# byteowlz/kokorox

Hardware: NVIDIA B200
Metric: audio-seconds per second (higher is better)
Workload: dtype bf16

## Files before the change

kokorox_b200/csrc/capi.cu:

```cuda
#include "../../include/kkx.h"
#include "../../include/kkx_test.h"
#include "model.h"
#include <chrono>
#include <condition_variable>
#include <cstring>
#include <deque>
#include <mutex>
#include <map>
#include <numeric>
#include <set>
#include <sstream>
#include <atomic>
#include <thread>

using namespace kkx;

struct kkx_ctx {
  std::unique_ptr<Model> model;
  std::mutex mu;
  std::mutex pool_mu;
  std::map<float*, size_t> pinned;
  std::vector<std::pair<float*, size_t>> pinned_free;
  size_t pinned_free_floats = 0;
  size_t pinned_hi = 0;
// ... 445 lines not shown
    if (law != 0 && law != 1) throw ArgError("law must be 0 (mu-law) or 1 (A-law), got " + std::to_string(law));
    Model& m = *ctx->model;
    m.stage(batch, tokens, tok_offsets, styles, speeds);
    m.set_g711(law);
    try { m.run(); } catch (...) { m.set_g711(-1); throw; }
    m.set_g711(-1);
    const long long n = m.total_samples();
    size_t cap = 0;
    float* host = take_pinned(ctx, (size_t)(n + 3) / 4, &cap);
    try {
      m.fetch_g711(reinterpret_cast<unsigned char*>(host), n, out_sample_offsets, out_pred_dur);
    } catch (...) { cudaFreeHost(host); throw; }
    hand_out(ctx, host, cap);
    *out_codes = reinterpret_cast<uint8_t*>(host);
  });
}

KKX_API void kkx_release_g711(kkx_ctx* ctx, uint8_t* codes) { kkx_release(ctx, reinterpret_cast<float*>(codes)); }

KKX_API int kkx_infer_batch_flac(kkx_ctx* ctx, int32_t batch, const int64_t* tokens, const int32_t* tok_offsets,
                                 const float* styles, const float* speeds, uint8_t** out_bytes,
                                 int64_t* out_byte_offsets, int64_t* out_sample_offsets, int32_t* out_pred_dur) {
  int rc = check_ctx(ctx);
  if (rc) return rc;
  if (out_bytes) *out_bytes = nullptr;
  std::lock_guard<std::mutex> lk(ctx->mu);
  return guarded(ctx, [&] {
    if (!out_bytes) throw ArgError("out_bytes is null");
    if (!out_byte_offsets) throw ArgError("out_byte_offsets is null");
    Model& m = *ctx->model;
    m.stage(batch, tokens, tok_offsets, styles, speeds);
    m.set_pcm16(true);
    try { m.run(); } catch (...) { m.set_pcm16(false); throw; }
    m.set_pcm16(false);
    m.encode_flac();
    const long long n = m.flac_bytes();
    size_t cap = 0;
    float* host = take_pinned(ctx, (size_t)(n + 3) / 4, &cap);
    try {
      m.fetch_flac(reinterpret_cast<unsigned char*>(host), n, out_byte_offsets, out_sample_offsets, out_pred_dur);
    } catch (...) { cudaFreeHost(host); throw; }
    hand_out(ctx, host, cap);
    *out_bytes = reinterpret_cast<uint8_t*>(host);
  });
}

KKX_API void kkx_release_flac(kkx_ctx* ctx, uint8_t* bytes) { kkx_release(ctx, reinterpret_cast<float*>(bytes)); }

static void put_u16(uint8_t* p, uint32_t v) { p[0] = (uint8_t)v; p[1] = (uint8_t)(v >> 8); }
static void put_u32(uint8_t* p, uint32_t v) { put_u16(p, v & 0xFFFF); put_u16(p + 2, v >> 16); }
static void wav_header(uint8_t* h, uint32_t riff_size, uint32_t data_size, uint32_t format, uint32_t channels,
                       uint32_t rate, uint32_t bits) {
  memcpy(h, "RIFF", 4); put_u32(h + 4, riff_size); memcpy(h + 8, "WAVEfmt ", 8);
  put_u32(h + 16, 16); put_u16(h + 20, format); put_u16(h + 22, channels); put_u32(h + 24, rate);
  put_u32(h + 28, rate * channels * bits / 8); put_u16(h + 32, channels * bits / 8); put_u16(h + 34, bits);
  memcpy(h + 36, "data", 4); put_u32(h + 40, data_size);
}

KKX_API int32_t kkx_wav_header_pcm16(uint8_t* dst44, int64_t n_samples, int32_t sample_rate) {
  if (!dst44 || n_samples < 0 || sample_rate <= 0) return KKX_ERR_ARG;
  const uint32_t bytes = (uint32_t)(n_samples * 2);
  wav_header(dst44, 36u + bytes, bytes, 1, 1, (uint32_t)sample_rate, 16);
  return 44;
}

KKX_API int32_t kkx_wav_header_f32_stream(uint8_t* dst44, int32_t channels, int32_t sample_rate) {
  if (!dst44 || channels <= 0 || sample_rate <= 0) return KKX_ERR_ARG;
  wav_header(dst44, 0xFFFFFFFFu, 0xFFFFFFFFu, 3, (uint32_t)channels, (uint32_t)sample_rate, 32);
  return 44;
}

KKX_API int64_t kkx_encode_wav16_base64(const int16_t* pcm, int64_t n_samples, int32_t sample_rate, char* dst,
                                int64_t capacity) {
  if (n_samples < 0 || sample_rate <= 0 || (!pcm && n_samples > 0)) return KKX_ERR_ARG;
  const int64_t nbytes = 44 + n_samples * 2;
  const int64_t nchars = (nbytes + 2) / 3 * 4;
  if (!dst || capacity < nchars) return nchars;
  static const char T[] = "ABCDEFGHIJKLMNOPQRSTUVWXYZabcdefghijklmnopqrstuvwxyz0123456789+/";
  uint8_t head[48];
  kkx_wav_header_pcm16(head, n_samples, sample_rate);
  const uint8_t* body = reinterpret_cast<const uint8_t*>(pcm);
  const int64_t nbody = n_samples * 2;
  const int borrow = (int)std::min<int64_t>(4, nbody);
  for (int i = 0; i < borrow; i++) head[44 + i] = body[i];
  const int hbytes = 44 + borrow;
  char* o = dst;
  auto group = [&](const uint8_t* p, int n) {
    const uint32_t v = ((uint32_t)p[0] << 16) | ((n > 1 ? (uint32_t)p[1] : 0u) << 8) | (n > 2 ? (uint32_t)p[2] : 0u);
    o[0] = T[v >> 18]; o[1] = T[(v >> 12) & 63];
    o[2] = n > 1 ? T[(v >> 6) & 63] : '=';
    o[3] = n > 2 ? T[v & 63] : '=';
    o += 4;
  };
  int hp = 0;
  for (; hp + 3 <= hbytes; hp += 3) group(head + hp, 3);
  if (hp < hbytes) {
    group(head + hp, hbytes - hp);
  } else {
    int64_t bp = borrow;
    for (; bp + 3 <= nbody; bp += 3) group(body + bp, 3);
    if (bp < nbody) group(body + bp, (int)(nbody - bp));
  }
  if (capacity > nchars) *o = 0;
  return nchars;
}

KKX_API int kkx_infer(kkx_ctx* ctx, const int64_t* tokens, int32_t n_tokens, const float* style256,
              float speed, float** out_audio, int64_t* out_samples, int32_t* out_pred_dur) {
  if (out_samples) *out_samples = 0;
  if (ctx && ctx->model && ctx->coalesce_max.load() > 1) {
    if (out_audio) *out_audio = nullptr; else { g_err = "out_audio is null"; return KKX_ERR_ARG; }
    const int vrc = validate_request(tokens, n_tokens, style256, speed);
    if (vrc != KKX_OK) return vrc;
    kkx_ctx::Waiter w{tokens, n_tokens, style256, speed, out_pred_dur};
    const int rc = infer_coalesced(ctx, w);
    if (rc == KKX_OK) { *out_audio = w.audio; if (out_samples) *out_samples = w.samples; }
    return rc;
  }
  const int32_t offs[2] = {0, n_tokens};
  int64_t soff[2] = {0, 0};
  const int rc = kkx_infer_batch(ctx, 1, tokens, offs, style256, &speed, out_audio, soff, out_pred_dur);
  if (rc == KKX_OK && out_samples) *out_samples = soff[1];
  return rc;
}

static void async_worker(kkx_ctx* ctx) {
  std::unique_lock<std::mutex> al(ctx->amu);
  for (;;) {
    ctx->acv_work.wait(al, [&] { return ctx->astop || !ctx->aqueue.empty(); });
    if (ctx->astop) {
      for (auto* r : ctx->aqueue) { r->w.rc = KKX_ERR_STATE; r->w.err = "session destroyed before the request ran"; r->done = true; }
      ctx->aqueue.clear();
      ctx->acv_done.notify_all();
      return;
    }
    std::vector<kkx_ctx::AsyncReq*> reqs;
    std::vector<kkx_ctx::Waiter*> batch;
    long long tok = 0;
    const size_t want = (size_t)std::max(ctx->async_batch.load(), 1);
    while (!ctx->aqueue.empty() && reqs.size() < want) {
      kkx_ctx::AsyncReq* r = ctx->aqueue.front();
      if (!reqs.empty() && tok + r->w.n > 64 * 512) break;
      tok += r->w.n;
      reqs.push_back(r);
      batch.push_back(&r->w);
      ctx->aqueue.pop_front();
    }
    al.unlock();
    try {
      serve_coalesced(ctx, batch, false);
    } catch (...) {
      for (auto* w : batch) { w->rc = KKX_ERR_CUDA; w->err = "internal error while serving an asynchronous batch"; w->audio = nullptr; }
    }
    al.lock();
    ctx->async_batches++;
    ctx->async_requests += (int64_t)reqs.size();
    for (auto* r : reqs) r->done = true;
    ctx->acv_done.notify_all();
  }
}

KKX_API int kkx_submit(kkx_ctx* ctx, const int64_t* tokens, int32_t n_tokens, const float* style256, float speed,
                       kkx_ticket* out_ticket) {
  int rc = check_ctx(ctx);
  if (rc) return rc;
  if (!out_ticket) { g_err = "out_ticket is null"; return KKX_ERR_ARG; }
  *out_ticket = 0;
  rc = validate_request(tokens, n_tokens, style256, speed);
  if (rc) return rc;
  try {
    std::unique_ptr<kkx_ctx::AsyncReq> r(new kkx_ctx::AsyncReq());
    r->tokens.assign(tokens, tokens + n_tokens);
    memcpy(r->style, style256, sizeof r->style);
    r->dur.assign((size_t)n_tokens, 0);
    r->w.tokens = r->tokens.data(); r->w.n = n_tokens; r->w.style = r->style; r->w.speed = speed;
    r->w.pred_dur = r->dur.data();
    std::lock_guard<std::mutex> al(ctx->amu);
    if (ctx->astop) { g_err = "Session is not initialized."; return KKX_ERR_STATE; }
    if (!ctx->worker_started) {
      ctx->worker = std::thread(async_worker, ctx);
      ctx->worker_started = true;
    }
    const int64_t t = ctx->next_ticket++;
    ctx->aqueue.push_back(r.get());
    ctx->tickets[t] = std::move(r);
    *out_ticket = t;
  } catch (const std::exception& e) { g_err = e.what(); return KKX_ERR_CUDA; }
  ctx->acv_work.notify_one();
  return KKX_OK;
}

KKX_API int kkx_poll(kkx_ctx* ctx, kkx_ticket ticket) {
  int rc = check_ctx(ctx);
  if (rc) return rc;
  std::lock_guard<std::mutex> al(ctx->amu);
  auto it = ctx->tickets.find(ticket);
  if (it == ctx->tickets.end() || it->second->taken) { g_err = "unknown ticket"; return KKX_ERR_ARG; }
  return it->second->done ? 1 : 0;
}

KKX_API int kkx_wait(kkx_ctx* ctx, kkx_ticket ticket, float** out_audio, int64_t* out_samples, int32_t* out_pred_dur) {
  int rc = check_ctx(ctx);
  if (rc) return rc;
  if (out_audio) *out_audio = nullptr;
  if (out_samples) *out_samples = 0;
  std::unique_ptr<kkx_ctx::AsyncReq> r;
  {
    std::unique_lock<std::mutex> al(ctx->amu);
    auto it = ctx->tickets.find(ticket);
    if (it == ctx->tickets.end() || it->second->taken) { g_err = "unknown ticket"; return KKX_ERR_ARG; }
    it->second->taken = true;
    kkx_ctx::AsyncReq* p = it->second.get();
    ctx->acv_done.wait(al, [&] { return p->done; });
    r = std::move(it->second);
    ctx->tickets.erase(it);
  }
  if (r->w.rc != KKX_OK) { g_err = r->w.err; return r->w.rc; }
  if (out_pred_dur) memcpy(out_pred_dur, r->dur.data(), r->dur.size() * sizeof(int32_t));
  if (out_samples) *out_samples = r->w.samples;
  if (out_audio) *out_audio = r->w.audio; else kkx_release(ctx, r->w.audio);
  return KKX_OK;
}

KKX_API void kkx_release(kkx_ctx* ctx, float* audio) {
  if (!ctx || !audio) return;
  float* to_free = nullptr;
  {
    std::lock_guard<std::mutex> pl(ctx->pool_mu);
    auto vit = ctx->views.find(audio);
    if (vit != ctx->views.end()) {
      kkx_ctx::SharedBuf* sb = vit->second;
      ctx->views.erase(vit);
      if (--sb->refs > 0) return;
      ctx->pinned[sb->base] = sb->cap;
      audio = sb->base;
      delete sb;
    }
    auto it = ctx->pinned.find(audio);
    if (it == ctx->pinned.end()) return;
    if (ctx->pinned_free.size() < 64 && ctx->pinned_free_floats + it->second <= (size_t(1) << 28)) {
      ctx->pinned_free.push_back({it->first, it->second});
      ctx->pinned_free_floats += it->second;
    } else {
      to_free = audio;
    }
    ctx->pinned.erase(it);
  }
  if (to_free) {
    if (ctx->model) cudaSetDevice(ctx->model->device());
    cudaFreeHost(to_free);
  }
}

KKX_API int kkx_stage_batch(kkx_ctx* ctx, int32_t batch, const int64_t* tokens, const int32_t* tok_offsets,
                    const float* styles, const float* speeds) {
  int rc = check_ctx(ctx);
  if (rc) return rc;
  std::lock_guard<std::mutex> lk(ctx->mu);
  return guarded(ctx, [&] { ctx->model->stage(batch, tokens, tok_offsets, styles, speeds); });
}

KKX_API int kkx_run_staged(kkx_ctx* ctx, int64_t* out_total_samples, int64_t* out_launches) {
  int rc = check_ctx(ctx);
  if (rc) return rc;
  std::lock_guard<std::mutex> lk(ctx->mu);
  return guarded(ctx, [&] {
    ctx->model->run();
    if (out_total_samples) *out_total_samples = ctx->model->total_samples();
    if (out_launches) *out_launches = ctx->model->stats.launches;
  });
}

KKX_API int kkx_fetch_staged(kkx_ctx* ctx, float* dst_audio, int64_t capacity, int64_t* out_sample_offsets,
                     int32_t* out_pred_dur) {
  int rc = check_ctx(ctx);
  if (rc) return rc;
  std::lock_guard<std::mutex> lk(ctx->mu);
  return guarded(ctx, [&] { ctx->model->fetch(dst_audio, capacity, out_sample_offsets, out_pred_dur); });
}

KKX_API int kkx_set_option(kkx_ctx* ctx, const char* key, int64_t value) {
  int rc = check_ctx(ctx);
  if (rc) return rc;
  std::lock_guard<std::mutex> lk(ctx->mu);
  return guarded(ctx, [&] {
    if (!key) throw ArgError("null key");
    Options& o = ctx->model->opt;
    const std::string k(key);
    if (k == "precision") { if (value < 0 || value > 1) throw ArgError("precision must be 0 or 1"); o.precision = (int)value; }
    else if (k == "noise_seed") o.noise_seed = (unsigned long long)value;
    else if (k == "max_frames") { if (value < 1) throw ArgError("max_frames must be >= 1"); o.max_frames = (int)value; }
    else if (k == "stft_replicate") o.stft_replicate = value ? 1 : 0;
    else if (k == "latency_graphs") o.latency_graphs = value ? 1 : 0;
    else if (k == "attention_umma") o.attention_umma = value ? 1 : 0;
    else if (k == "lstm_fast_gates") o.lstm_fast_gates = value ? 1 : 0;
    else if (k == "fuse_noise_stats") o.fuse_noise_stats = value ? 1 : 0;
    else if (k == "ups_phase_loop") o.ups_phase_loop = value < 0 ? 0 : value > 3 ? 3 : (int)value;
    else if (k == "split_f16") o.split_f16 = value ? 1 : 0;
    else if (k == "stream_bf16") o.stream_bf16 = value ? 1 : 0;
    else if (k == "fuse_phases") o.fuse_phases = value ? 1 : 0;
    else if (k == "gemm_pair") o.gemm_pair = value ? 1 : 0;
    else if (k == "fuse_planes") o.fuse_planes = value ? 1 : 0;
    else if (k == "conv_pair") o.conv_pair = value ? 1 : 0;
    else if (k == "fork_max_batch") { if (value < 0 || value > 512) throw ArgError("fork_max_batch must be in 0..512"); o.fork_max_batch = (int)value; }
    else if (k == "max_tokens") { if (value < 512) throw ArgError("max_tokens must be >= 512"); ctx->max_tokens = value; }
    else if (k == "coalesce") {
      if (value < 0 || value > kMaxCoalesce) throw ArgError("coalesce must be in 0..512");
      ctx->coalesce_max.store((int)value);
    } else if (k == "coalesce_wait_us") {
      if (value < 0 || value > 1000000) throw ArgError("coalesce_wait_us must be in 0..1000000");
      ctx->coalesce_wait_us.store((int)value);
    } else if (k == "async_batch") {
      if (value < 1 || value > kMaxCoalesce) throw ArgError("async_batch must be in 1..512");
      ctx->async_batch.store((int)value);
    } else if (k == "out_rate") {
      int U = 0, D = 0;
      if (value < 8000 || value > 48000 || !resample_ratio((int)value, &U, &D)) {
        const long long g = value > 0 ? std::gcd<long long>(value, 24000) : 1;
        throw ArgError("out_rate " + std::to_string(value) + " Hz is not supported: out_rate / 24000 reduces to U/D = " +
                       std::to_string(value / g) + "/" + std::to_string(24000 / g) +
                       "; accepted are 8000..48000 Hz with max(U, D) <= 320 (8000, 11025, 12000, 16000, 22050, 24000, "
                       "32000, 44100, 48000)");
      }
      o.out_rate = (int)value;
    }
    else throw ArgError("unknown option: " + k);
  });
}

KKX_API int64_t kkx_get_stat(kkx_ctx* ctx, const char* key) {
  if (check_ctx(ctx) || !key) return -1;
  std::lock_guard<std::mutex> lk(ctx->mu);
  const std::string k(key);
  if (k == "launches") return ctx->model->stats.launches;
  if (k == "last_frames") return ctx->model->last_frames;
  if (k == "gpu_us") return (int64_t)ctx->model->last_gpu_us;
  if (k == "precision") return ctx->model->opt.precision;
  if (k == "out_rate") return ctx->model->opt.out_rate;
  if (k == "coalesced_batches") return ctx->coalesced_batches;
  if (k == "coalesced_requests") return ctx->coalesced_requests;
  if (k == "coalesced_largest") return ctx->coalesced_largest;
  if (k == "graph_replays") return ctx->model->graph_replays;
  if (k == "frame_groups") return (int64_t)ctx->model->group_first().size();
  if (k.rfind("group_first:", 0) == 0) {
    const long g = atol(k.c_str() + 12);
    const auto& gf = ctx->model->group_first();
    return g >= 0 && g < (long)gf.size() ? gf[g] : -1;
  }
  if (k == "weights_sessions") return (int64_t)ctx->model->weight_sessions();
  if (k == "weights_bytes") return (int64_t)ctx->model->weight_set().device_bytes;
  if (k == "weights_from_onnx") return ctx->model->weight_set().format == "onnx" ? 1 : 0;
  {
    std::lock_guard<std::mutex> al(ctx->amu);
    if (k == "async_batches") return ctx->async_batches;
    if (k == "async_requests") return ctx->async_requests;
  }
  return -1;
}

KKX_API int kkx_profile_enable(kkx_ctx* ctx, int enable) {
  int rc = check_ctx(ctx);
  if (rc) return rc;
  std::lock_guard<std::mutex> lk(ctx->mu);
  ctx->model->stats.profile = enable != 0;
  return KKX_OK;
}

KKX_API int64_t kkx_profile_json(kkx_ctx* ctx, char* buf, int64_t capacity) {
  if (check_ctx(ctx)) return -1;
  std::lock_guard<std::mutex> lk(ctx->mu);
  std::ostringstream os;
  os << "{\"conv_flops\": " << ctx->model->stats.conv_flops << ", \"arb_flops\": " << ctx->model->stats.arb_flops
     << ", \"arb_bytes\": " << ctx->model->stats.arb_bytes << ", \"gpu_us\": " << ctx->model->last_gpu_us
     << ", \"kernels\": {";
  bool first = true;
  for (auto& kv : ctx->model->prof_) {
    if (!first) os << ", ";
    first = false;
    os << "\"" << kv.first << "\": [" << kv.second.first << ", " << kv.second.second << "]";
  }
  os << "}}";
  const std::string s = os.str();
  if (buf && capacity > 0) {
    const size_t n = std::min<size_t>(s.size(), (size_t)capacity - 1);
    memcpy(buf, s.data(), n);
    buf[n] = 0;
  }
  return (int64_t)s.size();
}

KKX_API int kkx_set_noise(kkx_ctx* ctx, const float* noise, int64_t n) {
  int rc = check_ctx(ctx);
  if (rc) return rc;
  std::lock_guard<std::mutex> lk(ctx->mu);
  return guarded(ctx, [&] { ctx->model->set_noise(noise, n); });
}

KKX_API int kkx_set_inject_item(kkx_ctx* ctx, int32_t item, const char* name, const void* data, int64_t count) {
  int rc = check_ctx(ctx);
  if (rc) return rc;
  std::lock_guard<std::mutex> lk(ctx->mu);
  return guarded(ctx, [&] {
    if (!name) throw ArgError("null name");
    ctx->model->set_inject(name, item, count > 0 ? data : nullptr, count);
  });
}

KKX_API int kkx_set_inject(kkx_ctx* ctx, const char* name, const void* data, int64_t count) {
  return kkx_set_inject_item(ctx, 0, name, data, count);
}

KKX_API int kkx_debug_enable(kkx_ctx* ctx, int enable) {
  int rc = check_ctx(ctx);
  if (rc) return rc;
  std::lock_guard<std::mutex> lk(ctx->mu);
  ctx->model->set_debug(enable != 0, -1);
  return KKX_OK;
}

KKX_API int kkx_debug_select(kkx_ctx* ctx, int enable, int32_t item) {
  int rc = check_ctx(ctx);
  if (rc) return rc;
  std::lock_guard<std::mutex> lk(ctx->mu);
  ctx->model->set_debug(enable != 0, item);
  return KKX_OK;
}

KKX_API int64_t kkx_debug_stage(kkx_ctx* ctx, const char* name, int32_t item, float* dst, int64_t capacity,
                        int64_t* rows, int64_t* cols) {
  if (check_ctx(ctx) || !name) return -1;
  std::lock_guard<std::mutex> lk(ctx->mu);
  const DebugStage* s = ctx->model->debug_stage(name, item);
  if (!s) { g_err = std::string("no such debug stage: ") + name; return -1; }
  if (rows) *rows = s->rows;
  if (cols) *cols = s->cols;
  const int64_t n = (int64_t)s->data.size();
  if (dst && capacity > 0) memcpy(dst, s->data.data(), (size_t)std::min(n, capacity) * sizeof(float));
  return n;
}

}
```

kokorox_b200/csrc/kernels.h:

```cpp
#pragma once
#include "common.h"
#include <cuda_bf16.h>

namespace kkx {

enum Act : int { ACT_NONE = 0, ACT_LRELU = 1, ACT_SNAKE = 2, ACT_GELU_NEW = 3 };

struct ConvArgs {
  const float* in = nullptr; int ldi = 0;
  const int* in_off = nullptr; const int* in_len = nullptr;
  const int* m_len = nullptr; int max_m = 0; int B = 1;
  long long sum_m = 0;
  const float* w = nullptr; const float* bias = nullptr;
  int Ci = 0, Co = 0, ks = 1, dil = 1, pad = 0, stride = 1;
  const float* pscale = nullptr; const float* pshift = nullptr; int pld = 0;
  int pact = ACT_NONE; float pslope = 0.f; const float* palpha = nullptr;
  float* out = nullptr; int ldo = 0; int ocol = 0; const int* out_off = nullptr;
  int ors = 1, oro = 0;
  int eact = ACT_NONE;
  const float* res = nullptr; int ldr = 0; int rcol = 0; const int* res_off = nullptr;
  int res_shift = 0;
  float oscale = 1.f; int accumulate = 0;
};
void launch_conv_f32(const ConvArgs& a, cudaStream_t st);

struct TcConvArgs {
  const void* tmA = nullptr;
  const void* tmB = nullptr;
  const void* tmA2 = nullptr;
  const void* tmB2 = nullptr;
  const void* tmB_c = nullptr;
  const void* tmB2_c = nullptr;
  int cluster = 1;
  int tf32 = 0;
  int nprod = 3;
  int f16 = 0;
  float wscale = 1.f;
  int eact = ACT_NONE;
  int Cpad = 0, Ci = 0, Co = 0, ks = 1, dil = 1, pad = 0;
  const int* in_off = nullptr; const int* m_len = nullptr; int max_m = 0; int B = 1; long long sum_m = 0;
  const float* bias = nullptr;
  float* out = nullptr; int ldo = 0; int ocol = 0; const int* out_off = nullptr; int ors = 1, oro = 0;
  const float* res = nullptr; int ldr = 0; int rcol = 0; const int* res_off = nullptr; int res_shift = 0;
  float oscale = 1.f; int accumulate = 0; int vec4 = 0;
  long long* timing = nullptr;
  const int* tile_start = nullptr; int ntiles_m = 0;
  int group_m = 1;
  void* out_hi = nullptr; void* out_lo = nullptr; int out_pl_ld = 0;
  void* attn_pl[6] = {nullptr, nullptr, nullptr, nullptr, nullptr, nullptr};
  int pair = 0;
  int force_kernel = 0;
  int nphase = 1;
  int phase_pad[10] = {0};
  int phase_oro[10] = {0};
  int phase_loop = 0;
  int debug = 0;
};
void launch_conv_tc(const TcConvArgs& a, cudaStream_t st);
bool conv_tc_takes_pair(const TcConvArgs& a);
void make_tmap_bf16(void* out_map, const void* ptr, long long inner, long long outer,
                    long long pitch_elems, int box_outer);
void make_tmap_f32(void* out_map, const void* ptr, long long inner, long long outer,
                   long long pitch_elems, int box_outer);
void make_tmap_f16(void* out_map, const void* ptr, long long inner, long long outer,
                   long long pitch_elems, int box_outer);
inline int tc_box_n(int Co) { return Co > 128 ? 256 : (Co > 64 ? 128 : 64); }
inline int tc_box_n_tf32(int Co) { return Co > 64 ? 128 : 64; }
void launch_apply_tf32(const float* x, int ldx, int C, const float* scale, const float* shift, int act,
                       float slope, float* out_hi, float* out_lo, int Cpad, int rows_total,
                       const int* off, const int* len, int B, int max_len, cudaStream_t st);
constexpr float kSplitF16Scale = 16.f;
float split_f16_host(const float* w, size_t n, unsigned short* hi, unsigned short* lo);
void launch_apply_f16x2(const float* x, int ldx, int C, const float* scale, const float* shift, int act,
                        float slope, void* out_hi, void* out_lo, int Cpad, int rows_total,
                        const int* off, const int* len, int B, int max_len, cudaStream_t st);
void launch_apply_bf16(const float* x, int ldx, int C, const float* scale, const float* shift, int act,
                       float slope, const float* alpha, void* out, int Cpad, int rows_total,
                       const int* off, const int* len, int B, int max_len, cudaStream_t st);
void launch_im2col_bf16(const float* in, int ldi, int C, int ks, int stride, int pad, void* out, int Cpad,
                        int rows_total, const int* in_off, const int* in_len, const int* out_off,
                        const int* out_len, int B, int max_out_len, cudaStream_t st, int force_generic = 0);
void launch_pool_up_bf16(const float* in, int ldi, const float* scale, const float* shift, float slope,
                         const float* w, const float* bias, int C, void* out, int Cpad, int rows_total,
                         const int* in_off, const int* in_len, const int* out_off, int B, int max_len,
                         cudaStream_t st);

struct ArbConvArgs {
  const void* x = nullptr; int in_bf16 = 0;
  const float* scale = nullptr; const float* shift = nullptr;
  const float* alpha = nullptr;
  const void* tmB = nullptr;
  int C = 0, ks = 1, dil = 1, pad = 0;
  const int* off = nullptr; const int* len = nullptr;
  const int* tile_start = nullptr;
  int B = 1; int total_tiles = 0; long long sum_m = 0;
  const float* bias = nullptr;
  __nv_bfloat16* out_bf16 = nullptr;
  float* out_f32 = nullptr;
  const float* res = nullptr; float oscale = 1.f; int accumulate = 0;
  int res_bf16 = 0;
  float* part = nullptr; int nchunk = 0;
  long long* timing = nullptr;
  int debug = 0;
  int post = 0, cout = 0, ldo = 0; float slope = 0.f;
};
int arb_tile_rows(int C, int ks);
bool arb_conv_supported(int C, int ks, int dil, int B);
void launch_arb_conv(const ArbConvArgs& a, cudaStream_t st);

struct LnArgs {
  const float* x = nullptr; int ldx = 0;
  const float* res = nullptr; int ldr = 0;
  const float* w = nullptr; const float* b = nullptr;
  const float* ada = nullptr; int ada_ld = 0; int ada_off = 0;
  float eps = 1e-5f; float slope = 1.f;
  float* out = nullptr; int ldo = 0; int ocol = 0;
  const int* off = nullptr; const int* len = nullptr; int B = 1; int max_len = 0; int C = 0;
  void* pl_hi = nullptr; void* pl_lo = nullptr; int pl_ld = 0;
};
void launch_layernorm(const LnArgs& a, cudaStream_t st);

void launch_albert_embed(const int* ids, const float* word, const float* pos, const float* type,
                         const float* lnw, const float* lnb, float* out, const int* off,
                         const int* len, int B, int max_len, cudaStream_t st);
void launch_embed_rows(const int* ids, const float* table, int C, float* out, int ldo,
                       const int* off, const int* len, int B, int max_len, cudaStream_t st);
void launch_bcast_cols(const float* vec, int ldv, int voff, int C, float* out, int ldo, int ocol,
                       const int* off, const int* len, int B, int max_len, cudaStream_t st);
void launch_copy_cols(const float* src, int lds, int scol, float* dst, int ldd, int dcol, int C,
                      const int* off, const int* len, int B, int max_len, cudaStream_t st);
void launch_add_rows(const float* a, const float* b, float* out, int C, const int* off,
                     const int* len, int B, int max_len, cudaStream_t st);
void launch_copy_row(float* u, int C, int dst_row, int src_row, const int* off, int B,
                     cudaStream_t st);

void launch_attention(const float* qkv, float* ctx, const int* off, const int* len, int B,
                      int max_len, cudaStream_t st);

size_t attention_umma_scratch_floats(int rows_total, int B);
void attention_timing_dump();
void launch_attention_umma(const float* qkv, float* scratch, float* ctx, const int* off, const int* len, int B,
                           int max_len, int rows_total, cudaStream_t st, bool planes_ready = false);
void attention_umma_planes(float* scratch, int rows_total, int B, void* (&pl)[6]);

void launch_lstm(const float* xproj, const float* whhT, float* out, int ldo, int ocol,
                 const int* off, const int* len, int B, cudaStream_t st, int variant = 1);

constexpr int kStatRows = 128;
void launch_colstats(const float* x, int ldx, int C, float* part, const int* off, const int* len,
                     int B, int max_len, cudaStream_t st, void* out_bf16 = nullptr);
void launch_add_rows_stats(const float* a, const float* b, float* out, int C, float* part, const int* off,
                           const int* len, int B, int max_len, cudaStream_t st, void* out_bf16 = nullptr);
void launch_pointwise_conv_stats(const float* x, int ldx, int Ci, const float* w, const float* bias, float* out, int Co,
                                 float* part, const int* off, const int* len, int B, int max_len, long long sum_m,
                                 cudaStream_t st);
void launch_adain_coef(const float* part, int C, int max_len, const int* len, const float* sty,
                       int sld, int soff, float eps, float* scale, float* shift, int B,
                       cudaStream_t st);

void launch_pool_up(const float* in, int ldi, const float* scale, const float* shift, float slope,
                    const float* w , const float* bias, int C, float* out, int ldo,
                    const int* in_off, const int* in_len, const int* out_off, int B, int max_len,
                    cudaStream_t st);

void launch_duration(const float* logits, int K, const float* speeds, int* pred_dur,
                     float* dur_float, const int* off, const int* len, int B, int max_len,
                     cudaStream_t st);
void launch_dur_scan(const int* pred_dur, int* cum, int cum_ld, int* total, const int* off,
                     const int* len, int B, cudaStream_t st);
void launch_expand_idx(const int* cum, int cum_ld, const int* tok_len, int* idx, const int* fr_off,
                       const int* fr_len, int B, int max_len, cudaStream_t st);
void launch_gather_rows(const float* in, int ldi, const int* in_off, const int* idx,
                        const int* fr_off, const int* fr_len, int C, float* out, int ldo, int ocol,
                        int B, int max_len, cudaStream_t st);

void launch_curve_conv(const float* x, const int* x_off, const int* x_len, const float* w3,
                       const float* bias, float* out, int ldo, int ocol, const int* out_off,
                       const int* out_len, int B, int max_len, cudaStream_t st);

void launch_sine_phase(const float* f0, const int* f0_off, const int* f0_len, float* phase,
                       const int* ph_off , int B, cudaStream_t st);
void launch_sine_source(const float* f0, const int* f0_off, const int* f0_len, const float* phase,
                        const int* ph_off, const float* noise ,
                        unsigned long long seed, const float* lin_w, const float* lin_b,
                        float* out, const long long* s_off, int B, long long max_samples,
                        cudaStream_t st);
void launch_stft(const float* x, const long long* s_off, float* har, int ldh, const int* h_off,
                 const int* h_len, int replicate_pad, int B, int max_len, cudaStream_t st);
void launch_istft(const float* cp, int ldc, const int* h_off, const int* h_len, float* audio, short* pcm ,
                  const long long* s_off, int fast, int B, int max_len, cudaStream_t st);

bool resample_ratio(int out_rate, int* U, int* D);
int resample_design(int out_rate, std::vector<float>* taps, int* U, int* D, int* H);
void launch_resample(const float* x, const long long* in_off, const long long* in_len, const long long* out_off,
                     const float* taps, int U, int D, int H, float* out, short* pcm ,
                     unsigned char* codes , int law, int B, long long max_out, cudaStream_t st);

long long flac_frames(long long n);
long long flac_bound(long long n_items, long long n_frames, long long n_samples);
size_t flac_work_bytes(long long n_frames);
bool flac_rate_ok(int rate);
void launch_flac(const short* pcm, const long long* soff, const int* foff, int B, int F, int rate, void* work,
                 unsigned char* out, long long* item_off, cudaStream_t st);

void launch_mix_styles(const float* table, const int* mix_off, const int* voice_ids, const float* portions,
                       const int* rows, float* styles, int B, cudaStream_t st);

}
```

kokorox_b200/csrc/kernels_arb.cu:

```cuda
#include "kernels.h"
#include "tc_ptx.cuh"
#include <type_traits>
#include <cstdlib>

namespace kkx {

namespace {

#ifdef KKX_ARB_TIMING
#define TIM_DECL(n) long long tim_acc[n] = {0}; long long tim_last = clock64(); const bool tim_on = a.timing && blockIdx.x == 0
#define TICK(slot) do { if (tim_on) { const long long now_ = clock64(); tim_acc[slot] += now_ - tim_last; tim_last = now_; } } while (0)
#define TIM_FLUSH(base, n) do { if (tim_on) for (int i_ = 0; i_ < (n); i_++) atomicAdd(reinterpret_cast<unsigned long long*>(a.timing) + (base) + i_, (unsigned long long)tim_acc[i_]); } while (0)
#else
#define TIM_DECL(n)
#define TICK(slot)
#define TIM_FLUSH(base, n)
#endif

#ifdef KKX_EXPERIMENTS
#define ARB_DBG(a, bit) ((a).debug & (bit))
#else
#define ARB_DBG(a, bit) (0)
#endif

constexpr int kArbThreads = 512;
constexpr int kArbMaxB = 512;

template <int BN, int MSUB, bool T>
struct ArbCfg {
  static constexpr int KCH = BN / 64;
  static constexpr int RA = MSUB * 128 + 56;
  static constexpr uint32_t A_SLOT = RA * 128;
  static constexpr int NA = (BN == 128 && (!T || MSUB == 4)) ? 2 : 3;
  static constexpr uint32_t B_STAGE = BN * 128;
  static constexpr int NB = (T && MSUB == 4) ? 4 : (BN == 128) ? 6 : 3;
  static constexpr int PITCH = 36;
  static constexpr uint32_t STG = T ? 0 : 2 * 128 * PITCH * 4;
  static constexpr uint32_t STAT = 4 * BN * 2 * 4;
  static constexpr uint32_t COEF = 3 * BN * 4;
  static constexpr int NBAR = 2 * NA + 2 * NB + 4;
  static constexpr uint32_t SMEM = NA * A_SLOT + NB * B_STAGE + STG + STAT + COEF + NBAR * 8 + 16 + (3 * kArbMaxB + 2) * 4 + 1024;
  static_assert(A_SLOT % 1024 == 0, "A slot must keep the 1024-byte swizzle alignment");
};

__device__ __forceinline__ uint32_t pack_bf16(float lo, float hi) {
  __nv_bfloat162 p = __floats2bfloat162_rn(lo, hi);
  return *reinterpret_cast<uint32_t*>(&p);
}

struct TileCur {
  int b, mt;
  __device__ __forceinline__ void init(const int* ts, int B, int tile) {
    int lo = 0, hi = B;
    while (hi - lo > 1) {
      const int mid = (lo + hi) >> 1;
      if (ts[mid] <= tile) lo = mid; else hi = mid;
    }
    b = lo; mt = tile - ts[lo];
  }
  __device__ __forceinline__ void next(const int* ts) {
    mt++;
    while (ts[b] + mt >= ts[b + 1]) { b++; mt = 0; if (ts[b] < 0) break; }
  }
};

template <int BN, int MSUB, bool CONV2, bool T, bool POST = false, int SB = 0, bool PB = false>
__global__ void __launch_bounds__(kArbThreads, 1) arb_conv_kernel(const __grid_constant__ CUtensorMap tmB, ArbConvArgs a) {
  static_assert(SB == 0 || (!POST && (CONV2 || SB == 1)), "stream-bf16 variants: conv1 SB=1, conv2 SB=1 (bf16 out) / SB=2 (fp32 out)");
  static_assert(!PB || (T && !CONV2 && !POST && SB == 0 && MSUB == 2), "balanced-producer variant: conv1, transposed accumulator, fp32 input");
  constexpr bool XIN_BF = CONV2 || SB != 0;
  constexpr bool OUT_BF = !CONV2 || SB == 1;
  static_assert(!T || (BN == 128 && (MSUB == 2 || MSUB == 4)), "transposed mode: C = 128, 256- or 512-row tiles");
  static_assert(!POST || (T && !CONV2 && MSUB == 2), "post variant: transposed accumulator, fp32 input");
  constexpr int NBUF = (T && MSUB == 4) ? 1 : 2;
  constexpr int NEW = PB ? 4 : 8;
  constexpr int NPW = PB ? 8 : 14 - NEW;
  constexpr int kProdThreads = NPW * 32;
  constexpr int kProdRows = kProdThreads / 8;
  using Cfg = ArbCfg<BN, MSUB, T>;
  constexpr int KCH = Cfg::KCH, NA = Cfg::NA, NB = Cfg::NB, PITCH = Cfg::PITCH;
  constexpr int MT = MSUB * 128;
  extern __shared__ uint8_t smem_raw[];
  const uint32_t base = (smem_u32(smem_raw) + 1023u) & ~1023u;
  uint8_t* const gbase = smem_raw + (base - smem_u32(smem_raw));
  const uint32_t a_base = base;
  const uint32_t b_base = a_base + NA * Cfg::A_SLOT;
  const uint32_t stg_base = b_base + NB * Cfg::B_STAGE;
  const uint32_t stat_base = stg_base + Cfg::STG;
  const uint32_t coef_base = stat_base + Cfg::STAT;
  const uint32_t bar_base = coef_base + Cfg::COEF;
  const uint32_t tmem_slot = bar_base + Cfg::NBAR * 8;
  const uint32_t ts_base = tmem_slot + 16;
  auto fullA = [&](int s) { return bar_base + s * 8; };
  auto emptyA = [&](int s) { return bar_base + (NA + s) * 8; };
  auto fullB = [&](int s) { return bar_base + (2 * NA + s) * 8; };
  auto emptyB = [&](int s) { return bar_base + (2 * NA + NB + s) * 8; };
  auto tfull = [&](int j) { return bar_base + (2 * NA + 2 * NB + j) * 8; };
  auto tempty = [&](int j) { return bar_base + (2 * NA + 2 * NB + 2 + j) * 8; };
  int* const s_ts = reinterpret_cast<int*>(gbase + (ts_base - base));
  int* const s_len = s_ts + (kArbMaxB + 2);
  int* const s_off = s_len + kArbMaxB;

  const int warp = threadIdx.x >> 5, lane = threadIdx.x & 31;
  const int B = a.B;
#pragma unroll 1
  for (int i = threadIdx.x; i <= B + 1; i += kArbThreads) s_ts[i] = i <= B ? a.tile_start[i] : -1;
#pragma unroll 1
  for (int i = threadIdx.x; i < B; i += kArbThreads) { s_len[i] = a.len[i]; s_off[i] = a.off[i]; }

  if (warp == 0 && lane == 0) {
    asm volatile("prefetch.tensormap [%0];" ::"l"(&tmB) : "memory");
    for (int s = 0; s < NA; s++) { mbar_init(fullA(s), kProdThreads / 32); mbar_init(emptyA(s), 1); }
    for (int s = 0; s < NB; s++) { mbar_init(fullB(s), 1); mbar_init(emptyB(s), 1); }
    for (int j = 0; j < 2; j++) { mbar_init(tfull(j), 1); mbar_init(tempty(j), NEW); }
    asm volatile("fence.mbarrier_init.release.cluster;" ::: "memory");
    asm volatile("fence.proxy.async.shared::cta;" ::: "memory");
  }
  if (warp == 1) {
    asm volatile("tcgen05.alloc.cta_group::1.sync.aligned.shared::cta.b32 [%0], %1;" ::"r"(tmem_slot), "r"(512u) : "memory");
    asm volatile("tcgen05.relinquish_alloc_permit.cta_group::1.sync.aligned;" ::: "memory");
  }
  tc_fence_before();
  __syncthreads();
  tc_fence_after();
  uint32_t tmem_base;
  asm volatile("ld.shared.b32 %0, [%1];" : "=r"(tmem_base) : "r"(tmem_slot) : "memory");

  const int t_begin = (int)(((long long)a.total_tiles * blockIdx.x) / gridDim.x);
  const int t_end = (int)(((long long)a.total_tiles * (blockIdx.x + 1)) / gridDim.x);
  const int ks = a.ks, dil = a.dil, pad = a.pad;

  if (warp == 0) {
    if (lane == 0 && t_begin < t_end) {
      int g = 0;
      TIM_DECL(2);
      const bool resident = KCH * ks <= NB;
#pragma unroll 1
      for (int tile = t_begin; tile < (resident ? t_begin + 1 : t_end); tile++) {
#pragma unroll 1
        for (int c = 0; c < KCH; c++)
#pragma unroll 1
          for (int tap = 0; tap < ks; tap++, g++) {
            const int s = g % NB;
            mbar_wait(emptyB(s), (((uint32_t)(g / NB)) & 1u) ^ 1u);
            TICK(0);
            mbar_expect_tx(fullB(s), Cfg::B_STAGE);
            tma_load_2d(b_base + s * Cfg::B_STAGE, &tmB, tap * BN + c * 64, 0, fullB(s));
            TICK(1);
          }
      }
      TIM_FLUSH(0, 2);
    }
  } else if (warp == 1) {
    if (lane == 0 && t_begin < t_end) {
      constexpr uint32_t idesc = umma_idesc_bf16(128, BN);
      int gA = 0, gB = 0, ti = 0;
      TileCur cur;
      cur.init(s_ts, B, t_begin);
      const bool resident = KCH * ks <= NB;
      TIM_DECL(4);
#pragma unroll 1
      for (int tile = t_begin; tile < t_end; tile++, ti++) {
        const int rem = s_len[cur.b] - cur.mt * MT;
        (void)rem;
        const int buf = NBUF == 2 ? (ti & 1) : 0;
        mbar_wait(tempty(buf), (NBUF == 2 ? (((uint32_t)(ti >> 1)) & 1u) : ((uint32_t)ti & 1u)) ^ 1u);
        tc_fence_after();
        TICK(0);
#pragma unroll 1
        for (int c = 0; c < KCH; c++, gA++) {
          const int sa = gA % NA;
          mbar_wait(fullA(sa), ((uint32_t)(gA / NA)) & 1u);
          tc_fence_after();
          TICK(1);
          const uint32_t slot = a_base + sa * Cfg::A_SLOT;
#pragma unroll 1
          for (int tap = 0; tap < ks; tap++, gB++) {
            const int sb = resident ? c * ks + tap : gB % NB;
            if (!resident || ti == 0) {
              mbar_wait(fullB(sb), resident ? 0u : ((uint32_t)(gB / NB)) & 1u);
              tc_fence_after();
            }
            TICK(2);
            const uint64_t bd = umma_desc_sw128(b_base + sb * Cfg::B_STAGE);
            if (T) {
              constexpr uint32_t idescT = umma_idesc_bf16(128, 256);
              const uint64_t wd = bd;
#pragma unroll
              for (int s2 = 0; s2 < MSUB / 2; s2++) {
                const uint64_t xd = umma_desc_sw128(slot + (uint32_t)(s2 * 256 + tap * dil) * 128u);
                const uint32_t td = tmem_base + (uint32_t)(buf * 256 + s2 * 256);
#pragma unroll
                for (int k = 0; k < 4; k++)
                  if (!ARB_DBG(a, 8)) umma_bf16(td, wd + (uint64_t)(2 * k), xd + (uint64_t)(2 * k), idescT, (c | tap | k) ? 1u : 0u);
              }
            } else {
#pragma unroll
              for (int sub = 0; sub < MSUB; sub++) {
                if (sub * 128 >= rem) continue;
                const uint64_t ad = umma_desc_sw128(slot + (uint32_t)(sub * 128 + tap * dil) * 128u);
                const uint32_t td = tmem_base + (uint32_t)((buf * MSUB + sub) * BN);
#pragma unroll
                for (int k = 0; k < 4; k++)
                  umma_bf16(td, ad + (uint64_t)(2 * k), bd + (uint64_t)(2 * k), idesc, (c | tap | k) ? 1u : 0u);
              }
            }
            if (!resident) umma_commit(emptyB(sb));
            TICK(3);
          }
          umma_commit(emptyA(sa));
        }
        umma_commit(tfull(buf));
        cur.next(s_ts);
      }
      TIM_FLUSH(4, 4);
    }
  } else if (T && warp < 2 + NEW) {
    const int eg = (warp - 2) >> 2;
    const int q = warp & 3;
    const int co = q * 32 + lane;
    const float bias_c = a.bias[co];
    const float2 bias2 = make_float2(bias_c, bias_c);
    const float2 os2 = make_float2(a.oscale, a.oscale);
    const bool accum = a.accumulate != 0;
    constexpr int RW = MSUB * 128 / (NEW / 4);
    constexpr int NCHK = RW / 32;
    auto fetchT = [&](int L, int off, int m0, int ch, float (&rv)[32]) {
      if (!CONV2 || ARB_DBG(a, 2)) return;
      const int row = m0 + eg * RW + ch * 32;
      const int left = L - row;
      if (SB) {
        const __nv_bfloat16* rp = reinterpret_cast<const __nv_bfloat16*>(a.res) + (size_t)(off + row) * 128 + co;
#pragma unroll
        for (int j = 0; j < 32; j++)
          if (j < left) rv[j] = __bfloat162float(rp[j * 128]);
      } else {
        const float* rp = a.res + (size_t)(off + row) * 128 + co;
#pragma unroll
        for (int j = 0; j < 32; j++)
          if (j < left) {
            if (ARB_DBG(a, 32)) asm volatile("ld.global.L1::no_allocate.f32 %0, [%1];" : "=f"(rv[j]) : "l"(rp + j * 128));
            else rv[j] = rp[j * 128];
          }
      }
    };
    int ti = 0;
    TileCur cur;
    float rv0[32], rv1[32];
    if (t_begin < t_end) {
      cur.init(s_ts, B, t_begin);
      fetchT(s_len[cur.b], s_off[cur.b], cur.mt * MT, 0, rv0);
      fetchT(s_len[cur.b], s_off[cur.b], cur.mt * MT, 1, rv1);
    }
#ifdef KKX_ARB_TIMING
    long long tim_acc[9] = {0}; long long tim_last = clock64();
    const bool tim_on = a.timing && blockIdx.x == 0 && warp == 2 && lane == 0;
#endif
#pragma unroll 1
    for (int tile = t_begin; tile < t_end; tile++, ti++) {
      const int b = cur.b;
      const int L = s_len[b], off = s_off[b];
      const int m0 = cur.mt * MT;
      const int buf = NBUF == 2 ? (ti & 1) : 0;
      cur.next(s_ts);
      const bool has_next = tile + 1 < t_end;
      const int nL = has_next ? s_len[cur.b] : 0, noff = has_next ? s_off[cur.b] : 0, nm0 = cur.mt * MT;
      TICK(8);
      mbar_wait(tfull(buf), NBUF == 2 ? (((uint32_t)(ti >> 1)) & 1u) : ((uint32_t)ti & 1u));
      tc_fence_after();
      TICK(0);
      float2 s2 = make_float2(0.f, 0.f), q2 = s2;
      auto bodyT = [&](int ch, float (&rv)[32], auto full_tag) {
        constexpr bool FULL = decltype(full_tag)::value;
        const int row = m0 + eg * RW + ch * 32;
        const int left = ARB_DBG(a, 2) ? 0 : L - row;
        uint32_t v[32];
        tmem_ld32(tmem_base + ((uint32_t)(q * 32) << 16) + (uint32_t)(buf * 256 + eg * RW + ch * 32), v);
        if (ch == NCHK - 1) {
          tc_fence_before();
          if (lane == 0) asm volatile("mbarrier.arrive.shared::cta.b64 _, [%0];" ::"r"(tempty(buf)) : "memory");
        }
        TICK(1);
        if (CONV2 && !OUT_BF) {
          float* op = a.out_f32 + (size_t)(off + row) * 128 + co;
#pragma unroll
          for (int j = 0; j < 32; j += 2) {
            float2 o = make_float2(__uint_as_float(v[j]), __uint_as_float(v[j + 1]));
            o = __fadd2_rn(__fadd2_rn(o, make_float2(rv[j], rv[j + 1])), bias2);
            if (!FULL) { o.x = j < left ? o.x : 0.f; o.y = j + 1 < left ? o.y : 0.f; }
            s2 = __fadd2_rn(s2, o);
            q2 = __ffma2_rn(o, o, q2);
            o = __fmul2_rn(o, os2);
            if (accum) {
              if (FULL || j < left) asm volatile("red.global.add.f32 [%0], %1;" ::"l"(op + j * 128), "f"(o.x) : "memory");
              if (FULL || j + 1 < left) asm volatile("red.global.add.f32 [%0], %1;" ::"l"(op + (j + 1) * 128), "f"(o.y) : "memory");
            } else {
              if (FULL || j < left) op[j * 128] = o.x;
              if (FULL || j + 1 < left) op[(j + 1) * 128] = o.y;
            }
          }
        } else if (POST) {
          if (co < a.cout) {
            float* op = a.out_f32 + (size_t)(off + row) * a.ldo + co;
#pragma unroll
            for (int j = 0; j < 32; j++)
              if (FULL || j < left) op[(size_t)j * a.ldo] = __uint_as_float(v[j]) + bias_c;
          }
        } else {
          const int odd = lane & 1;
          __nv_bfloat16* op = a.out_bf16 + (size_t)(off + row + odd) * 128 + (co & ~1);
#pragma unroll
          for (int j = 0; j < 32; j += 2) {
            float2 o = make_float2(__uint_as_float(v[j]), __uint_as_float(v[j + 1]));
            if (CONV2) o = __fadd2_rn(o, make_float2(rv[j], rv[j + 1]));
            o = __fadd2_rn(o, bias2);
            if (!FULL) { o.x = j < left ? o.x : 0.f; o.y = j + 1 < left ? o.y : 0.f; }
            s2 = __fadd2_rn(s2, o);
            q2 = __ffma2_rn(o, o, q2);
            const float send = odd ? o.x : o.y;
            const float recv = __shfl_xor_sync(0xffffffffu, send, 1);
            const uint32_t w = odd ? pack_bf16(recv, o.y) : pack_bf16(o.x, recv);
            if (FULL || j + odd < left) *reinterpret_cast<uint32_t*>(op + j * 128) = w;
          }
        }
        TICK(5);
        if (ch + 2 < NCHK) fetchT(L, off, m0, ch + 2, rv);
        else if (has_next) fetchT(nL, noff, nm0, ch + 2 - NCHK, rv);
        TICK(6);
        if ((ch & 3) == 3) {
          if (a.part && row - 96 < L) {
            float* pp = a.part + ((size_t)b * a.nchunk + (size_t)((row - 96) >> 7)) * 2 * 128 + co;
            pp[0] = s2.x + s2.y;
            pp[128] = q2.x + q2.y;
          }
          s2 = make_float2(0.f, 0.f); q2 = s2;
        }
      };
      if (L - m0 >= MT && !ARB_DBG(a, 2)) {
#pragma unroll
        for (int ch = 0; ch < NCHK; ch += 2) { bodyT(ch, rv0, std::true_type{}); bodyT(ch + 1, rv1, std::true_type{}); }
      } else {
#pragma unroll
        for (int ch = 0; ch < NCHK; ch += 2) { bodyT(ch, rv0, std::false_type{}); bodyT(ch + 1, rv1, std::false_type{}); }
      }
      TICK(7);
    }
    TIM_FLUSH(8, 9);
  } else if (!T && warp < 10) {
    const int eg = (warp - 2) >> 2;
    const int q = warp & 3;
    const int et = q * 32 + lane;
    const int t = (threadIdx.x - 64) & 127;
    const int tr = t >> 3;
    const int c4 = (t & 7) << 2;
    const int bar_id = 1 + eg;
    float* const buf_f = reinterpret_cast<float*>(gbase + (stg_base - base)) + eg * (128 * PITCH);
    float* const stat_f = reinterpret_cast<float*>(gbase + (stat_base - base));
    const float* const st_rd = buf_f + tr * PITCH + c4;
    float* const st_wr = buf_f + et * PITCH;
    constexpr int NCH = BN / 64;
    constexpr int RS = 16 * BN;
    const float2 os2 = make_float2(a.oscale, a.oscale);
    const bool accum = a.accumulate != 0;
    auto fetch = [&](int L, int off, int m0, int e, float4 (&rv)[8]) {
      if (!CONV2) return;
      const int sub = e / NCH, ci = e & (NCH - 1);
      const int row = m0 + sub * 128 + tr;
      const int left = L - row;
      if (SB) {
        const __nv_bfloat16* rp = reinterpret_cast<const __nv_bfloat16*>(a.res) + (size_t)(off + row) * BN + ((2 * ci + eg) * 32 + c4);
#pragma unroll
        for (int i = 0; i < 8; i++)
          if (16 * i < left) {
            const uint2 w = *reinterpret_cast<const uint2*>(rp + i * RS);
            rv[i] = make_float4(__uint_as_float(w.x << 16), __uint_as_float(w.x & 0xFFFF0000u),
                                __uint_as_float(w.y << 16), __uint_as_float(w.y & 0xFFFF0000u));
          }
      } else {
        const float* rp = a.res + (size_t)(off + row) * BN + ((2 * ci + eg) * 32 + c4);
#pragma unroll
        for (int i = 0; i < 8; i++)
          if (16 * i < left) rv[i] = *reinterpret_cast<const float4*>(rp + i * RS);
      }
    };
    int ti = 0;
    TileCur cur;
    float4 rv0[8], rv1[8];
#ifdef KKX_ARB_TIMING
    long long tim_acc[9] = {0}; long long tim_last = clock64();
    const bool tim_on = a.timing && blockIdx.x == 0 && warp == 2 && lane == 0;
#endif
    if (t_begin < t_end) {
      cur.init(s_ts, B, t_begin);
      fetch(s_len[cur.b], s_off[cur.b], cur.mt * MT, 0, rv0);
      fetch(s_len[cur.b], s_off[cur.b], cur.mt * MT, 1, rv1);
    }
#pragma unroll 1
    for (int tile = t_begin; tile < t_end; tile++, ti++) {
      const int b = cur.b;
      const int L = s_len[b], off = s_off[b];
      const int m0 = cur.mt * MT;
      const int nsub = min(MSUB, (L - m0 + 127) >> 7);
      const int E = nsub * NCH;
      const int buf = ti & 1;
      cur.next(s_ts);
      const bool has_next = tile + 1 < t_end;
      const int nL = has_next ? s_len[cur.b] : 0, noff = has_next ? s_off[cur.b] : 0, nm0 = cur.mt * MT;
      TICK(8);
      mbar_wait(tfull(buf), ((uint32_t)(ti >> 1)) & 1u);
      tc_fence_after();
      TICK(0);
      auto body = [&](int e, float4 (&rv)[8], auto full_tag) {
        constexpr bool FULL = decltype(full_tag)::value;
        const int sub = e / NCH, ci = e & (NCH - 1);
        const int row = m0 + sub * 128 + tr;
        const int n = (2 * ci + eg) * 32 + c4;
        {
          uint32_t v[32];
          tmem_ld32(tmem_base + ((uint32_t)(q * 32) << 16) + (uint32_t)((buf * MSUB + sub) * BN + n - c4), v);
          if (e == E - 1) {
            tc_fence_before();
            if (lane == 0) asm volatile("mbarrier.arrive.shared::cta.b64 _, [%0];" ::"r"(tempty(buf)) : "memory");
          }
          TICK(1);
          asm volatile("bar.sync %0, 128;" ::"r"(bar_id) : "memory");
          TICK(2);
#pragma unroll
          for (int j = 0; j < 32; j += 4)
            *reinterpret_cast<uint4*>(st_wr + j) = make_uint4(v[j], v[j + 1], v[j + 2], v[j + 3]);
          TICK(3);
        }
        asm volatile("bar.sync %0, 128;" ::"r"(bar_id) : "memory");
        TICK(4);
        const float4 bb = *reinterpret_cast<const float4*>(a.bias + n);
        const float2 b01 = make_float2(bb.x, bb.y), b23 = make_float2(bb.z, bb.w);
        const int left = L - row;
        const size_t g0 = (size_t)(off + row) * BN + n;
        float2 s01 = make_float2(0.f, 0.f), s23 = s01, q01 = s01, q23 = s01;
#pragma unroll
        for (int i = 0; i < 8; i++) {
          const bool ok = FULL || 16 * i < left;
          const float4 ov = *reinterpret_cast<const float4*>(st_rd + i * 16 * PITCH);
          float2 o01 = make_float2(ov.x, ov.y), o23 = make_float2(ov.z, ov.w);
          if (CONV2) { o01 = __fadd2_rn(o01, make_float2(rv[i].x, rv[i].y)); o23 = __fadd2_rn(o23, make_float2(rv[i].z, rv[i].w)); }
          o01 = __fadd2_rn(o01, b01); o23 = __fadd2_rn(o23, b23);
          if (!FULL) { o01.x = ok ? o01.x : 0.f; o01.y = ok ? o01.y : 0.f; o23.x = ok ? o23.x : 0.f; o23.y = ok ? o23.y : 0.f; }
          s01 = __fadd2_rn(s01, o01); s23 = __fadd2_rn(s23, o23);
          q01 = __ffma2_rn(o01, o01, q01); q23 = __ffma2_rn(o23, o23, q23);
          if (OUT_BF) {
            uint2 pk;
            pk.x = pack_bf16(o01.x, o01.y); pk.y = pack_bf16(o23.x, o23.y);
            if (ok) *reinterpret_cast<uint2*>(a.out_bf16 + g0 + i * RS) = pk;
          } else {
            o01 = __fmul2_rn(o01, os2); o23 = __fmul2_rn(o23, os2);
            float* op = a.out_f32 + g0 + i * RS;
            if (ok) {
              if (accum)
                asm volatile("red.global.add.v4.f32 [%0], {%1, %2, %3, %4};" ::"l"(op), "f"(o01.x), "f"(o01.y), "f"(o23.x), "f"(o23.y) : "memory");
              else
                *reinterpret_cast<float4*>(op) = make_float4(o01.x, o01.y, o23.x, o23.y);
            }
          }
        }
        TICK(5);
        if (e + 2 < E) fetch(L, off, m0, e + 2, rv);
        else if (has_next) fetch(nL, noff, nm0, e + 2 - E, rv);
        TICK(6);
        if (a.part) {
#pragma unroll
          for (int d = 8; d <= 16; d <<= 1) {
            float2 t0, t1, t2, t3;
            t0.x = __shfl_xor_sync(0xffffffffu, s01.x, d); t0.y = __shfl_xor_sync(0xffffffffu, s01.y, d);
            t1.x = __shfl_xor_sync(0xffffffffu, s23.x, d); t1.y = __shfl_xor_sync(0xffffffffu, s23.y, d);
            t2.x = __shfl_xor_sync(0xffffffffu, q01.x, d); t2.y = __shfl_xor_sync(0xffffffffu, q01.y, d);
            t3.x = __shfl_xor_sync(0xffffffffu, q23.x, d); t3.y = __shfl_xor_sync(0xffffffffu, q23.y, d);
            s01 = __fadd2_rn(s01, t0); s23 = __fadd2_rn(s23, t1); q01 = __fadd2_rn(q01, t2); q23 = __fadd2_rn(q23, t3);
          }
          if (lane < 8) {
            float* sp = stat_f + ((size_t)(t >> 5) * BN + n) * 2;
            *reinterpret_cast<float4*>(sp) = make_float4(s01.x, q01.x, s01.y, q01.y);
            *reinterpret_cast<float4*>(sp + 4) = make_float4(s23.x, q23.x, s23.y, q23.y);
          }
          if (ci == NCH - 1) {
            asm volatile("bar.sync %0, 128;" ::"r"(bar_id) : "memory");
            if (t < BN / 2) {
              const int nn = ((t >> 5) * 2 + eg) * 32 + (t & 31);
              float* pp = a.part + ((size_t)b * a.nchunk + (size_t)((m0 >> 7) + sub)) * 2 * BN + nn;
              const float* sf = stat_f + 2 * nn;
              pp[0] = (sf[0] + sf[2 * BN]) + (sf[4 * BN] + sf[6 * BN]);
              pp[BN] = (sf[1] + sf[2 * BN + 1]) + (sf[4 * BN + 1] + sf[6 * BN + 1]);
            }
          }
        }
        TICK(7);
      };
      if (L - m0 >= MT) {
#pragma unroll 1
        for (int e = 0; e < E; e += 2) {
          body(e, rv0, std::true_type{});
          body(e + 1, rv1, std::true_type{});
        }
        continue;
      }
#pragma unroll 1
      for (int e = 0; e < E; e += 2) {
        body(e, rv0, std::false_type{});
        body(e + 1, rv1, std::false_type{});
      }
    }
    TIM_FLUSH(8, 9);
  } else if (warp < 2 + NEW + NPW) {
    const int pt = threadIdx.x - (2 + NEW) * 32;
    const int cg = pt & 7;
    const int rl = pt >> 3;
    constexpr int GP = PB ? 3 : 4;
    constexpr int GR = GP * kProdRows;
    const int ra_used = MT + 2 * pad;
    const int ngc = (ra_used + GR - 1) / GR;
    float* const coef = reinterpret_cast<float*>(gbase + (coef_base - base));
    const int F = (t_end - t_begin) * KCH * ngc;
    using Raw = typename std::conditional<XIN_BF, uint4, float4>::type;
    constexpr int RPP = XIN_BF ? 1 : 2;
    constexpr int XE = XIN_BF ? 2 : 4;
    const uint32_t sw = (uint32_t)rl * 128u + (uint32_t)((cg ^ (rl & 7)) << 4);

    TileCur lc; int l_c = 0, l_g = 0;
    TileCur sc_; int s_c = 0, s_g = 0, gA = 0, coef_b = -1;
    if (F > 0) { lc.init(s_ts, B, t_begin); sc_ = lc; }
    float2 cA[4], cB[4], cI[4];
#ifdef KKX_ARB_TIMING
    long long tim_acc[5] = {0}; long long tim_last = clock64();
    const bool tim_on = a.timing && blockIdx.x == 0 && warp == 10 && lane == 0;
#endif

    auto issue = [&](Raw (&rb)[GP][RPP]) {
      const int L = s_len[lc.b];
      const int row = lc.mt * MT - pad + l_g * GR + rl;
      const int rloc = l_g * GR + rl;
      const char* xp = reinterpret_cast<const char*>(a.x) + ((size_t)(s_off[lc.b] + row) * BN + (l_c * 64 + cg * 8)) * XE;
#pragma unroll
      for (int p = 0; p < GP; p++) {
        if ((unsigned)(row + p * kProdRows) < (unsigned)L && rloc + p * kProdRows < ra_used && !ARB_DBG(a, 1)) {
#pragma unroll
          for (int v = 0; v < RPP; v++) {
            const char* gp = xp + (size_t)p * kProdRows * BN * XE + v * 16;
            if (ARB_DBG(a, 16)) {
              uint4 t;
              asm volatile("ld.global.L1::no_allocate.v4.u32 {%0, %1, %2, %3}, [%4];" : "=r"(t.x), "=r"(t.y), "=r"(t.z), "=r"(t.w) : "l"(gp));
              rb[p][v] = *reinterpret_cast<Raw*>(&t);
            } else rb[p][v] = *reinterpret_cast<const Raw*>(gp);
          }
        }
      }
      if (++l_g == ngc) { l_g = 0; if (++l_c == KCH) { l_c = 0; lc.next(s_ts); } }
    };
    auto process = [&](Raw (&rb)[GP][RPP]) {
      const int b = sc_.b;
      const int sa = gA % NA;
      if (s_g == 0) {
        if (!POST && b != coef_b) {
          asm volatile("bar.sync 3, %0;" ::"n"(kProdThreads) : "memory");
          for (int ch = pt; ch < BN; ch += kProdThreads) {
            const float al = a.alpha[ch], s = a.scale[(size_t)b * BN + ch], h = a.shift[(size_t)b * BN + ch];
            coef[ch] = al * s; coef[BN + ch] = al * h; coef[2 * BN + ch] = 1.0f / al;
          }
          asm volatile("bar.sync 3, %0;" ::"n"(kProdThreads) : "memory");
          coef_b = b;
        }
        const float* cp = coef + s_c * 64 + cg * 8;
#pragma unroll
        for (int e = 0; !POST && e < 4; e += 2) {
          const float4 t0 = *reinterpret_cast<const float4*>(cp + 2 * e);
          const float4 t1 = *reinterpret_cast<const float4*>(cp + BN + 2 * e);
          const float4 t2 = *reinterpret_cast<const float4*>(cp + 2 * BN + 2 * e);
          cA[e] = make_float2(t0.x, t0.y); cA[e + 1] = make_float2(t0.z, t0.w);
          cB[e] = make_float2(t1.x, t1.y); cB[e + 1] = make_float2(t1.z, t1.w);
          cI[e] = make_float2(t2.x, t2.y); cI[e + 1] = make_float2(t2.z, t2.w);
        }
        TICK(1);
        mbar_wait(emptyA(sa), (((uint32_t)(gA / NA)) & 1u) ^ 1u);
        TICK(2);
      }
      const int L = s_len[b];
      const int row = sc_.mt * MT - pad + s_g * GR + rl;
      const int rloc = s_g * GR + rl;
      uint8_t* const sp = gbase + (a_base - base) + (size_t)sa * Cfg::A_SLOT + (size_t)(s_g * GR) * 128 + sw;
#pragma unroll
      for (int p = 0; p < GP; p++) {
        const uint32_t inmask = (unsigned)(row + p * kProdRows) < (unsigned)L ? 0xFFFFFFFFu : 0u;
        float2 xv[4];
        if (XIN_BF) {
          const uint4 raw = *reinterpret_cast<const uint4*>(&rb[p][0]);
          xv[0] = make_float2(__uint_as_float(raw.x << 16), __uint_as_float(raw.x & 0xFFFF0000u));
          xv[1] = make_float2(__uint_as_float(raw.y << 16), __uint_as_float(raw.y & 0xFFFF0000u));
          xv[2] = make_float2(__uint_as_float(raw.z << 16), __uint_as_float(raw.z & 0xFFFF0000u));
          xv[3] = make_float2(__uint_as_float(raw.w << 16), __uint_as_float(raw.w & 0xFFFF0000u));
        } else {
          const float4 f0 = *reinterpret_cast<const float4*>(&rb[p][0]);
          const float4 f1 = *reinterpret_cast<const float4*>(&rb[p][RPP - 1]);
          xv[0] = make_float2(f0.x, f0.y); xv[1] = make_float2(f0.z, f0.w);
          xv[2] = make_float2(f1.x, f1.y); xv[3] = make_float2(f1.z, f1.w);
        }
        uint32_t pw[4];
#pragma unroll
        for (int e = 0; e < 4; e++) {
          if (POST) {
            const float2 lx = __fmul2_rn(xv[e], make_float2(a.slope, a.slope));
            pw[e] = pack_bf16(fmaxf(xv[e].x, lx.x), fmaxf(xv[e].y, lx.y)) & inmask;
            continue;
          }
          if (ARB_DBG(a, 4)) { pw[e] = pack_bf16(xv[e].x, xv[e].y) & inmask; continue; }
          const float2 u = __ffma2_rn(xv[e], cA[e], cB[e]);
          const float2 sn = make_float2(__sinf(u.x), __sinf(u.y));
          const float2 y = __fmul2_rn(__ffma2_rn(sn, sn, u), cI[e]);
          pw[e] = pack_bf16(y.x, y.y) & inmask;
        }
        const uint4 pk = make_uint4(pw[0], pw[1], pw[2], pw[3]);
        if (rloc + p * kProdRows < ra_used) *reinterpret_cast<uint4*>(sp + p * kProdRows * 128) = pk;
      }
      TICK(3);
      if (++s_g == ngc) {
        asm volatile("fence.proxy.async.shared::cta;" ::: "memory");
        __syncwarp();
        if (lane == 0) asm volatile("mbarrier.arrive.shared::cta.b64 _, [%0];" ::"r"(fullA(sa)) : "memory");
        s_g = 0; gA++;
        if (++s_c == KCH) { s_c = 0; sc_.next(s_ts); }
      }
    };

    Raw bufA[GP][RPP], bufB[GP][RPP];
#pragma unroll
    for (int p = 0; p < GP; p++)
#pragma unroll
      for (int v = 0; v < RPP; v++) { bufA[p][v] = Raw(); bufB[p][v] = Raw(); }
    if (F > 0) issue(bufA);
#pragma unroll 1
    for (int f = 0; f < F; f += 2) {
      if (f + 1 < F) issue(bufB);
      TICK(0);
      process(bufA);
      if (f + 1 >= F) break;
      if (f + 2 < F) issue(bufA);
      TICK(0);
      process(bufB);
    }
    TIM_FLUSH(20, 5);
  }
  tc_fence_before();
  __syncthreads();
  if (warp == 1) {
    tc_fence_after();
    asm volatile("tcgen05.dealloc.cta_group::1.sync.aligned.b32 %0, %1;" ::"r"(tmem_base), "r"(512u) : "memory");
  }
}

template <int BN, int MSUB, bool CONV2, bool T, bool POST = false, int SB = 0, bool PB = false>
void launch_arb_t(const ArbConvArgs& a, cudaStream_t st) {
  using Cfg = ArbCfg<BN, MSUB, T>;
  static DevOnce once;
  int dev = 0;
  cudaGetDevice(&dev);
  once.run(dev, [] { KKX_CUDA(cudaFuncSetAttribute(arb_conv_kernel<BN, MSUB, CONV2, T, POST, SB, PB>, cudaFuncAttributeMaxDynamicSharedMemorySize, (int)Cfg::SMEM)); });
  const int nsm = device_sm_count(dev);
  const int grid = a.total_tiles < nsm ? a.total_tiles : nsm;
  arb_conv_kernel<BN, MSUB, CONV2, T, POST, SB, PB><<<grid, kArbThreads, Cfg::SMEM, st>>>(*reinterpret_cast<const CUtensorMap*>(a.tmB), a);
}

}

static int arb_variant(int C, int ks) {
  static const bool no_t = env_flag("KKX_ARB_NOT", false);
  static const bool use_512 = env_flag("KKX_ARB_512", false);
  if (C != 128 || no_t) return 0;
  return (ks >= 7 && use_512) ? 2 : 1;
}
int arb_tile_rows(int C, int ks) { return C == 128 ? (arb_variant(C, ks) == 2 ? 512 : 256) : 128; }

bool arb_conv_supported(int C, int ks, int dil, int B) {
  return (C == 128 || C == 256) && ks >= 1 && dil >= 1 && dil * (ks - 1) <= 50 && (ks & 1) && B <= kArbMaxB;
}

void launch_arb_conv(const ArbConvArgs& a, cudaStream_t st) {
  if (g_dry_run) return;
  if (a.total_tiles <= 0 || a.B <= 0) return;
  if (!arb_conv_supported(a.C, a.ks, a.dil, a.B)) throw ArgError("launch_arb_conv: unsupported shape");
  if (a.post) {
    if (a.C != 128 || a.in_bf16 || !a.out_f32 || a.out_bf16 || a.res || a.accumulate || a.part || a.cout < 1 || a.cout > 128 ||
        a.ldo < a.cout || !(a.slope > 0.f && a.slope < 1.f))
      throw ArgError("launch_arb_conv: unsupported post-conv arguments");
    if (g_launch_stats) g_launch_stats->conv_flops += 2.0 * (double)a.sum_m * a.C * a.cout * a.ks;
    launch_arb_t<128, 2, false, true, true>(a, st);
    post_launch("post_conv", st);
    return;
  }
  const bool conv2 = a.res != nullptr;
  if (conv2 ? (!a.in_bf16 || (a.out_f32 != nullptr) == (a.out_bf16 != nullptr) || (a.out_bf16 && (!a.res_bf16 || a.accumulate)))
            : (!a.out_bf16 || a.out_f32 || a.accumulate || a.res_bf16))
    throw ArgError("launch_arb_conv: unsupported input/output combination");
  const int variant = arb_variant(a.C, a.ks);
#ifdef KKX_EXPERIMENTS
  static const int dbg = env_int("KKX_ARB_DBG", 0);
  if (dbg && !a.debug) { ArbConvArgs d = a; d.debug = dbg; launch_arb_conv(d, st); return; }
#endif
  const bool stream_bf = conv2 ? a.res_bf16 != 0 : a.in_bf16 != 0;
  if (stream_bf && !(variant == 1 || a.C == 256)) throw ArgError("launch_arb_conv: the bf16 stream needs the default kernel variants");
  if (g_launch_stats) {
    const double fl = 2.0 * (double)a.sum_m * a.C * a.C * a.ks;
    g_launch_stats->conv_flops += fl;
    g_launch_stats->arb_flops += fl;
    const double bytes = conv2 ? 2.0 + (a.res_bf16 ? 2.0 : 4.0) + (a.out_bf16 ? 2.0 : 4.0) : (a.in_bf16 ? 2.0 : 4.0) + 2.0;
    g_launch_stats->arb_bytes += (double)a.sum_m * a.C * bytes;
  }
  if (stream_bf) {
    if (a.C == 128) {
      if (!conv2) launch_arb_t<128, 2, false, true, false, 1>(a, st);
      else if (a.out_bf16) launch_arb_t<128, 2, true, true, false, 1>(a, st);
      else launch_arb_t<128, 2, true, true, false, 2>(a, st);
    } else {
      if (!conv2) launch_arb_t<256, 1, false, false, false, 1>(a, st);
      else if (a.out_bf16) launch_arb_t<256, 1, true, false, false, 1>(a, st);
      else launch_arb_t<256, 1, true, false, false, 2>(a, st);
    }
  } else if (variant == 2) {
    if (a.in_bf16) launch_arb_t<128, 4, true, true>(a, st); else launch_arb_t<128, 4, false, true>(a, st);
  } else if (variant == 1) {
    static const bool pb = env_flag("KKX_ARB_PB", true);
    if (a.in_bf16) launch_arb_t<128, 2, true, true>(a, st);
    else if (pb) launch_arb_t<128, 2, false, true, false, 0, true>(a, st);
    else launch_arb_t<128, 2, false, true>(a, st);
  } else if (a.C == 128) {
    if (a.in_bf16) launch_arb_t<128, 2, true, false>(a, st); else launch_arb_t<128, 2, false, false>(a, st);
  } else {
    if (a.in_bf16) launch_arb_t<256, 1, true, false>(a, st); else launch_arb_t<256, 1, false, false>(a, st);
  }
  if (g_launch_stats && g_launch_stats->profile && g_launch_stats->detail) {
    char nm[96]; snprintf(nm, sizeof nm, "arb_conv[c%d k%d d%d %s%s m%lld]", a.C, a.ks, a.dil, conv2 ? "conv2" : "conv1", stream_bf ? " sb" : "", a.sum_m);
    post_launch(nm, st);
  } else post_launch("arb_conv", st);
}

}
```

kokorox_b200/csrc/model.h:

```cpp
#pragma once
#include "common.h"
#include "kernels.h"
#include <deque>
#include <functional>
#include <map>
#include <memory>
#include <mutex>
#include <string>
#include <tuple>
#include <vector>

namespace kkx {

struct HostTensor {
  std::vector<int> shape;
  const float* data = nullptr;
  size_t numel = 0;
};

class WeightFile {
 public:
  explicit WeightFile(const std::string& path);
  const HostTensor& get(const std::string& name) const;
  bool has(const std::string& name) const { return t_.count(name) != 0; }
  void put(const std::string& name, const std::vector<int>& shape, std::vector<float>&& data);
  void erase(const std::string& name) { t_.erase(name); }
  std::vector<std::string> names() const;
  const std::string& format() const { return format_; }

 private:
  void load_kkxw(const std::string& path);
  std::vector<char> buf_;
  std::deque<std::vector<float>> owned_;
  std::map<std::string, HostTensor> t_;
  std::string format_;
};
void load_onnx_weights(const std::string& path, const std::vector<char>& bytes, WeightFile& out);
std::vector<std::pair<std::string, std::vector<int>>> kokoro_tensor_specs();

struct TcW {
  void* w = nullptr;
  alignas(64) unsigned char tmap[128];
  alignas(64) unsigned char tmap_h[128];
  bool has_h = false;
  const void* pair_map(int co_tile) const { return co_tile >= 256 && co_tile % 256 == 0 && has_h ? tmap_h : nullptr; }
  int Cpad = 0, Ci = 0, Co = 0, ks = 0;
};
struct TcW32 {
  float* hi = nullptr; float* lo = nullptr;
  alignas(64) unsigned char tm_hi[128];
  alignas(64) unsigned char tm_lo[128];
  alignas(64) unsigned char tm_hi_c[128];
  alignas(64) unsigned char tm_lo_c[128];
  bool has_c = false;
  int Cpad = 0, Ci = 0, Co = 0, ks = 0;
  void* h_hi = nullptr; void* h_lo = nullptr;
  alignas(64) unsigned char tm16_hi[128];
  alignas(64) unsigned char tm16_lo[128];
  alignas(64) unsigned char tm16_hi_c[128];
  alignas(64) unsigned char tm16_lo_c[128];
  float wscale16 = 1.f;
};
struct LstmW { float* wih = nullptr; float* bias = nullptr; float* whhT = nullptr; int in = 0; TcW32 t_ih; };
struct AdaBlkW {
  int ci = 0, co = 0; bool up = false;
  float *w1 = nullptr, *b1 = nullptr, *w2 = nullptr, *b2 = nullptr, *w1x1 = nullptr;
  float *poolw = nullptr, *poolb = nullptr;
  int sty1 = 0, sty2 = 0;
  TcW t1, t2, t1x1;
  TcW32 s1, s2, s1x1;
};
struct ArbW {
  int c = 0, k = 0;
  float *w1[3], *b1[3], *w2[3], *b2[3], *a1[3], *a2[3];
  int s1[3], s2[3];
  TcW t1[3], t2[3];
};

struct Weights {
  float *word, *pos, *type, *emb_lnw, *emb_lnb, *map_w, *map_b;
  float *qkv_w, *qkv_b, *dense_w, *dense_b, *attn_lnw, *attn_lnb;
  float *ffn_w, *ffn_b, *ffo_w, *ffo_b, *full_lnw, *full_lnb;
  float *benc_w, *benc_b;
  TcW32 t_map, t_qkv, t_dense, t_ffn, t_ffo, t_benc, t_durp, t_tcnn[3];
  LstmW dur_lstm[3]; int dur_ada[3];
  LstmW pred_lstm, shared_lstm;
  float *durp_w, *durp_b;
  AdaBlkW f0blk[3], nblk[3];
  float *f0proj_w, *f0proj_b, *nproj_w, *nproj_b;
  float* temb; float *tcnn_w[3], *tcnn_b[3], *tln_g[3], *tln_b[3]; LstmW te_lstm;
  AdaBlkW enc, dec[4];
  float *f0conv_w, *f0conv_b, *nconv_w, *nconv_b, *asr_w, *asr_b;
  float *lin_w, *lin_b, *nc0_w, *nc0_b, *nc1_w, *nc1_b;
  ArbW nres[2], res[6];
  std::vector<float*> ups0, ups1;
  std::vector<TcW> tups0, tups1;
  TcW tups0_all, tups1_all;
  TcW t_post, t_nc0, t_nc1, t_asr;
  float *ups0_b, *ups1_b, *post_w, *post_b;
  TcW t_post_arb; float* post_b128 = nullptr;
  float *sty_pro_w, *sty_pro_b, *sty_dec_w, *sty_dec_b;
  int sty_pro_n = 0, sty_dec_n = 0;
};

void arb_timing_dump();

struct DebugStage { std::vector<float> data; long long rows = 0, cols = 0; };

struct Options {
  int precision = 1;
  unsigned long long noise_seed = 0x5eed;
  int max_frames = 49152;
  int stft_replicate = 0;
  int latency_graphs = 1;
  int fork_max_batch = 4;
  int attention_umma = 1;
  int split_f16 = 1;
  int stream_bf16 = 0;
  int fuse_phases = 1;
  int gemm_pair = 1;
  int fuse_planes = 1;
  int conv_pair = 1;
  int fuse_noise_stats = 1;
  int ups_phase_loop = 3;
  int lstm_fast_gates = 1;
  int out_rate = 24000;
};

class WeightSet {
 public:
  static std::shared_ptr<const WeightSet> acquire(const std::string& path, int device);
  ~WeightSet();
  WeightSet(const WeightSet&) = delete;
  WeightSet& operator=(const WeightSet&) = delete;
  Weights W;
  int device = 0;
  size_t device_bytes = 0;
  std::string format;

 private:
  WeightSet() = default;
  void load(const WeightFile& wf);
  float* up(const std::vector<float>& v);
  TcW make_tc(const std::vector<float>& w_co_ks_ci, int Co, int ks, int Ci);
  TcW32 make_tc32(const std::vector<float>& w_co_ks_ci, int Co, int ks, int Ci);
  std::vector<void*> owned_;
};

constexpr float kMinSpeed = 0.1f, kMaxSpeed = 10.f;
constexpr int kMaxItemFrames = 65536;

class Model {
 public:
  Model(const std::string& weights_path, int device);
  ~Model();

  void stage(int B, const int64_t* tokens, const int32_t* tok_offsets, const float* styles,
             const float* speeds);
  void load_voices(const float* table, int n_voices);
  void stage_voices(int B, const int64_t* tokens, const int32_t* tok_offsets, const int32_t* mix_offsets,
                    const int32_t* voice_ids, const float* portions, const int32_t* style_rows, const float* speeds);
  void set_pcm16(bool on) { want_pcm_ = on; }
  void fetch_pcm16(short* dst, long long capacity, int64_t* sample_offsets, int32_t* pred_dur);
  void set_g711(int law) { want_law_ = law; }
  void fetch_g711(unsigned char* dst, long long capacity, int64_t* sample_offsets, int32_t* pred_dur);
  void encode_flac();
  long long flac_bytes() const { return flac_valid_ ? flac_off_.back() : 0; }
  void fetch_flac(unsigned char* dst, long long capacity, int64_t* byte_offsets, int64_t* sample_offsets,
                  int32_t* pred_dur);
  std::function<float*(long long)> host_sink;
  bool sink_filled() const { return sink_filled_; }
  void run();
  long long total_samples() const { return total_samples_; }
  void fetch(float* dst, long long capacity, int64_t* sample_offsets, int32_t* pred_dur);

  void set_noise(const float* noise, long long n);
  void set_inject(const std::string& name, int item, const void* data, long long count);
  void set_debug(bool on, int item = -1) { debug_ = on; debug_item_ = item; }
  const DebugStage* debug_stage(const std::string& name, int item) const;
  const std::vector<int>& group_first() const { return group_first_; }

  Options opt;
  LaunchStats stats;
  long long last_frames = 0;
  double last_gpu_us = 0;
  std::map<std::string, std::pair<long long, double>> prof_;
  int device() const { return device_; }
  cudaStream_t stream() const { return stream_; }
  const WeightSet& weight_set() const { return *ws_; }
  long weight_sessions() const { return ws_.use_count(); }

 private:
  struct Run {
    float* d = nullptr;
    float* t_en = nullptr;
    float* sty_pro = nullptr;
    float* sty_dec = nullptr;
    int* pred_dur = nullptr;
    int* cum = nullptr;
    int* total = nullptr;
    std::vector<int> T;
    Level styL;
  };
  struct GemmPlanes {
    const void* in_hi = nullptr; const void* in_lo = nullptr;
    void* out_hi = nullptr; void* out_lo = nullptr; int out_ld = 0; bool out_done = false;
    float* attn_scratch = nullptr;
  };
  void gemm(const Level& Lin, const Level& Lm, const float* in, int ldi, int K, const float* w, const TcW32* w32,
            const float* bias, int N, float* out, int ldo, int ocol, int eact = ACT_NONE, int ks = 1,
            int pad = 0, const float* pscale = nullptr, const float* pshift = nullptr, int pact = ACT_NONE,
            float pslope = 0.f, const float* res = nullptr, int ldr = 0, const Level* Lres = nullptr,
            int res_shift = 0, float oscale = 1.f, GemmPlanes* pl = nullptr);
  bool planes_ok() const { return opt.precision == 1 && opt.split_f16 && opt.fuse_planes; }
  float* split_hi_ = nullptr; float* split_lo_ = nullptr; size_t split_cap_ = 0;
  struct Lane { float* hi = nullptr; float* lo = nullptr; size_t cap = 0; };
  Lane lane_[2];
  int lane_id_ = 0;
  void set_lane_scratch(int i, float* hi, float* lo, size_t cap) { lane_[i].hi = hi; lane_[i].lo = lo; lane_[i].cap = cap; if (i == lane_id_) use_lane(i); }
  void use_lane(int i) {
    lane_id_ = i; cur_ = i ? stream2_ : stream_;
    split_hi_ = lane_[i].hi; split_lo_ = lane_[i].lo; split_cap_ = lane_[i].cap;
  }
  void fork_lane1();
  void join_lane1();
  bool can_fork(int B) const { return B <= opt.fork_max_batch && !debug_ && !stats.profile && !stats.check_each; }
  void tc_conv(Arena& A, const void* abuf, int rows_total, const TcW& w, int dil, int pad, const Level& Lin,
               const Level& Lm, const float* bias, float* out, int ldo, int ocol, const Level& Lout, int ors,
               int oro, const float* res, int ldr, const Level* Lres, int res_shift, float oscale,
               bool accumulate);
  void token_phase(Run& r);
  void token_issue(Run& r);
  void token_finish(Run& r);
  size_t token_arena_bytes() const;
  void frame_phase(Run& r, int b0, int b1, bool dry);
  void adain_blk(Run& r, Arena& A, const AdaBlkW& w, const float* x, int ldx, const Level& Lin,
                 const Level& Lout, const float* sty, int sld, float* out, int ldo, int ocol,
                 bool dry);
  void arb(Run& r, Arena& A, const ArbW& w, const float* x, const Level& L, const float* sty,
           int sld, float* xw, float* t1, float* out, float oscale, bool accumulate,
           const float* part_x = nullptr, const void* x_bf16 = nullptr);
  bool use_stream_bf16(int C, int k, int B) const;
  Level make_level(const std::vector<int>& lens, Arena& A, int first_off = kGapRows);
  void upload(void* dst, const void* src, size_t bytes);
  void capture(const char* name, const float* p, int ld, int col, int cols, const Level& L,
               int item0);
  bool want_debug(int item) const { return debug_ && (debug_item_ < 0 || debug_item_ == item); }

  int device_ = 0;
  std::shared_ptr<const WeightSet> ws_;
  const Weights& W;
  cudaStream_t stream_ = nullptr;
  cudaStream_t stream2_ = nullptr;
  cudaStream_t cur_ = nullptr;
  cudaEvent_t ev_fork_ = nullptr, ev_join_ = nullptr;
  struct GraphKey {
    int n_tokens, precision; const void *tok_base, *io_ids, *io_level, *h_T, *h_dur;
    bool operator<(const GraphKey& o) const {
      return std::tie(n_tokens, precision, tok_base, io_ids, io_level, h_T, h_dur) <
             std::tie(o.n_tokens, o.precision, o.tok_base, o.io_ids, o.io_level, o.h_T, o.h_dur);
    }
  };
  struct GraphEntry { cudaGraphExec_t exec = nullptr; Run run; long long launches = 0; };
  std::map<GraphKey, GraphEntry> graphs_;
  PinnedArena graph_pin_;
  bool capturing_ = false;
  void clear_graphs();
 public:
  long long graph_replays = 0;
 private:
  Arena tokA_, frA_, ioA_;
  PinnedArena pin_;
  bool debug_ = false; int debug_item_ = -1;
  std::map<std::string, DebugStage> dbg_;
  int B_ = 0;
  bool staged_ = false, ran_ = false;
  std::vector<int> tok_len_;
  int* d_ids_ = nullptr; float* d_styles_ = nullptr; float* d_speeds_ = nullptr;
  Level tokL_;
  float* d_audio_ = nullptr; size_t audio_cap_ = 0;
  short* d_pcm_ = nullptr; size_t pcm_cap_ = 0; bool want_pcm_ = false, pcm_valid_ = false;
  unsigned char* d_g711_ = nullptr; size_t g711_cap_ = 0; int want_law_ = -1; bool g711_valid_ = false;
  unsigned char* d_flac_ = nullptr; size_t flac_cap_ = 0; bool flac_valid_ = false;
  char* d_flac_meta_ = nullptr; size_t flac_meta_cap_ = 0;
  std::vector<long long> flac_off_;
  bool resample_ = false; int rs_U_ = 1, rs_D_ = 1, rs_H_ = 0;
  float* d_taps_ = nullptr; int taps_rate_ = 0;
  void prepare_resample();
  float* d_voices_ = nullptr; int n_voices_ = 0;
  std::vector<long long> sample_off_;
  int* h_pred_dur_ = nullptr; size_t h_pred_dur_cap_ = 0;
  int* h_T_ = nullptr; size_t h_T_cap_ = 0;
  long long total_samples_ = 0;
  std::vector<int> group_first_;
  float* d_noise_ = nullptr; long long noise_n_ = 0;
  std::map<int, std::vector<int>> inj_dur_;
  std::map<int, std::vector<float>> inj_f0_, inj_n_;
  cudaEvent_t ev0_ = nullptr, ev1_ = nullptr;
  cudaStream_t copy_stream_ = nullptr; cudaEvent_t ev_grp_ = nullptr; bool sink_filled_ = false;
};

}
```

kokorox_b200/csrc/model_forward.cu:

```cuda
#include "model.h"
#include <algorithm>
#include <cmath>
#include <cstdlib>

namespace kkx {

namespace {
long long* g_arb_timing = nullptr;
long long* arb_timing_buf() {
  static const bool on = env_flag("KKX_ARB_TIMING", false);
  if (!on) return nullptr;
  if (!g_arb_timing) {
    KKX_CUDA(cudaMalloc(&g_arb_timing, 128 * sizeof(long long)));
    KKX_CUDA(cudaMemset(g_arb_timing, 0, 128 * sizeof(long long)));
  }
  return g_arb_timing;
}
ConvArgs gemm_args(const Level& L, const float* in, int ldi, int K, const float* w, const float* bias,
                   int N, float* out, int ldo, int ocol) {
  ConvArgs a;
  a.in = in; a.ldi = ldi; a.in_off = L.d_off; a.in_len = L.d_len;
  a.m_len = L.d_len; a.max_m = L.max_len; a.B = L.B; a.sum_m = L.sum_len;
  a.w = w; a.bias = bias; a.Ci = K; a.Co = N;
  a.out = out; a.ldo = ldo; a.ocol = ocol; a.out_off = L.d_off;
// ... 133 lines not shown
    const GraphKey key{tok_len_[0], opt.lstm_fast_gates * 32 + opt.precision * 16 + opt.attention_umma * 8 + opt.split_f16 * 4 + opt.gemm_pair * 2 + opt.fuse_planes, tokA_.base(), d_ids_, tokL_.d_off, h_T_, h_pred_dur_};
    auto it = graphs_.find(key);
    if (it != graphs_.end() && it->second.exec) {
      r = it->second.run;
      if (cudaGraphLaunch(it->second.exec, stream_) == cudaSuccess) {
        stats.launches += it->second.launches;
        graph_replays++;
        token_finish(r);
        return;
      }
      cudaGetLastError();
      cudaGraphExecDestroy(it->second.exec);
      graphs_.erase(it);
    } else if (it != graphs_.end()) {
      if (graphs_.size() > 64) clear_graphs();
      GraphEntry e;
      const long long l0 = stats.launches;
      cudaGraph_t g = nullptr;
      KKX_CUDA(cudaStreamBeginCapture(stream_, cudaStreamCaptureModeThreadLocal));
      capturing_ = true;
      token_issue(r);
      capturing_ = false;
      KKX_CUDA(cudaStreamEndCapture(stream_, &g));
      const cudaError_t ie = cudaGraphInstantiate(&e.exec, g, 0);
      cudaGraphDestroy(g);
      if (ie != cudaSuccess) { cudaGetLastError(); e.exec = nullptr; }
      e.run = r;
      e.launches = stats.launches - l0;
      if (e.exec && cudaGraphLaunch(e.exec, stream_) == cudaSuccess) {
        graphs_[key] = e;
        graph_replays++;
        token_finish(r);
        return;
      }
      cudaGetLastError();
      if (e.exec) cudaGraphExecDestroy(e.exec);
      graphs_.erase(key);
      stats.launches = l0;
    } else {
      graphs_[key] = GraphEntry();
    }
  }
  token_issue(r);
  token_finish(r);
}

void Model::token_issue(Run& r) {
  use_lane(0);
  cudaStream_t st = stream_;
  const Level& L = tokL_;
  const size_t R = (size_t)L.rows;
  const int B = B_;
  tokA_.reset();
  Arena& A = tokA_;
  const bool fork = can_fork(B);

  r.styL = make_level(std::vector<int>{B}, A, 0);
  r.sty_pro = A.alloc<float>((size_t)B * W.sty_pro_n);
  r.sty_dec = A.alloc<float>((size_t)B * W.sty_dec_n);
  launch_conv_f32(gemm_args(r.styL, d_styles_ + 128, 256, 128, W.sty_pro_w, W.sty_pro_b, W.sty_pro_n,
                            r.sty_pro, W.sty_pro_n, 0), st);
  launch_conv_f32(gemm_args(r.styL, d_styles_, 256, 128, W.sty_dec_w, W.sty_dec_b, W.sty_dec_n,
                            r.sty_dec, W.sty_dec_n, 0), st);

  {
    float* hi = A.alloc<float>(R * 2048); float* lo = A.alloc<float>(R * 2048);
    set_lane_scratch(0, hi, lo, R * 2048);
    float* hi1 = A.alloc<float>(R * 512); float* lo1 = A.alloc<float>(R * 512);
    set_lane_scratch(1, hi1, lo1, R * 512);
  }

  float* ta = A.alloc<float>(R * 512);
  float* tb = A.alloc<float>(R * 512);
  float* xp_te = A.alloc<float>(R * 2048);
  r.t_en = A.alloc<float>(R * 512);
  auto text_encoder = [&] {
    cudaStream_t ts = cur_;
    launch_embed_rows(d_ids_, W.temb, 512, ta, 512, L.d_off, L.d_len, B, L.max_len, ts);
    for (int i = 0; i < 3; i++) {
      gemm(L, L, ta, 512, 512, W.tcnn_w[i], &W.t_tcnn[i], W.tcnn_b[i], 512, tb, 512, 0, ACT_NONE, 5, 2);
      LnArgs ln;
      ln.x = tb; ln.ldx = 512; ln.w = W.tln_g[i]; ln.b = W.tln_b[i]; ln.eps = 1e-5f; ln.slope = 0.2f;
      ln.out = ta; ln.ldo = 512; ln.off = L.d_off; ln.len = L.d_len; ln.B = B; ln.max_len = L.max_len;
      ln.C = 512;
      launch_layernorm(ln, ts);
    }
    gemm(L, L, ta, 512, 512, W.te_lstm.wih, &W.te_lstm.t_ih, W.te_lstm.bias, 2048, xp_te, 2048, 0);
    launch_lstm(xp_te, W.te_lstm.whhT, r.t_en, 512, 0, L.d_off, L.d_len, B, ts, opt.precision != 0 && opt.lstm_fast_gates);
  };
  if (fork) {
    fork_lane1();
    use_lane(1);
    text_encoder();
    use_lane(0);
  }

  float* e = A.alloc<float>(R * 128);
  float* h = A.alloc<float>(R * 768);
  float* h1 = A.alloc<float>(R * 768);
  float* ctx = A.alloc<float>(R * 768);
  float* tmp = A.alloc<float>(R * 768);
  float* qkv = A.alloc<float>(R * 2304);
  float* ff = A.alloc<float>(R * 2048);
  float* att_scratch = opt.attention_umma ? A.alloc<float>(attention_umma_scratch_floats((int)R, B)) : nullptr;
  const bool pl_ok = planes_ok();
  void* p768h = pl_ok ? A.alloc_bytes(R * 768 * 2) : nullptr;
  void* p768l = pl_ok ? A.alloc_bytes(R * 768 * 2) : nullptr;
  void* p2048h = pl_ok ? A.alloc_bytes(R * 2048 * 2) : nullptr;
  void* p2048l = pl_ok ? A.alloc_bytes(R * 2048 * 2) : nullptr;
  bool h_planes = false;
  launch_albert_embed(d_ids_, W.word, W.pos, W.type, W.emb_lnw, W.emb_lnb, e, L.d_off, L.d_len, B,
                      L.max_len, st);
  gemm(L, L, e, 128, 128, W.map_w, &W.t_map, W.map_b, 768, h, 768, 0);
  for (int layer = 0; layer < 12; layer++) {
    GemmPlanes gq;
    if (h_planes) { gq.in_hi = p768h; gq.in_lo = p768l; }
    if (pl_ok && att_scratch) gq.attn_scratch = att_scratch;
    gemm(L, L, h, 768, 768, W.qkv_w, &W.t_qkv, W.qkv_b, 2304, qkv, 2304, 0, ACT_NONE, 1, 0, nullptr, nullptr, ACT_NONE, 0.f,
         nullptr, 0, nullptr, 0, 1.f, &gq);
    if (att_scratch) launch_attention_umma(qkv, att_scratch, ctx, L.d_off, L.d_len, B, L.max_len, L.rows, st, gq.out_done);
    else launch_attention(qkv, ctx, L.d_off, L.d_len, B, L.max_len, st);
    gemm(L, L, ctx, 768, 768, W.dense_w, &W.t_dense, W.dense_b, 768, tmp, 768, 0);
    LnArgs ln;
    ln.x = h; ln.ldx = 768; ln.res = tmp; ln.ldr = 768; ln.w = W.attn_lnw; ln.b = W.attn_lnb;
    ln.eps = 1e-12f; ln.out = h1; ln.ldo = 768; ln.off = L.d_off; ln.len = L.d_len; ln.B = B;
    ln.max_len = L.max_len; ln.C = 768;
    if (pl_ok) { ln.pl_hi = p768h; ln.pl_lo = p768l; ln.pl_ld = 768; }
    launch_layernorm(ln, st);
    GemmPlanes gf;
    if (pl_ok) { gf.in_hi = p768h; gf.in_lo = p768l; gf.out_hi = p2048h; gf.out_lo = p2048l; gf.out_ld = 2048; }
    gemm(L, L, h1, 768, 768, W.ffn_w, &W.t_ffn, W.ffn_b, 2048, ff, 2048, 0, ACT_GELU_NEW, 1, 0, nullptr, nullptr, ACT_NONE, 0.f,
         nullptr, 0, nullptr, 0, 1.f, &gf);
    GemmPlanes go;
    if (gf.out_done) { go.in_hi = p2048h; go.in_lo = p2048l; }
    gemm(L, L, ff, 2048, 2048, W.ffo_w, &W.t_ffo, W.ffo_b, 768, tmp, 768, 0, ACT_NONE, 1, 0, nullptr, nullptr, ACT_NONE, 0.f,
         nullptr, 0, nullptr, 0, 1.f, &go);
    ln.x = tmp; ln.res = h1; ln.w = W.full_lnw; ln.b = W.full_lnb; ln.out = h;
    launch_layernorm(ln, st);
    h_planes = pl_ok;
  }
  capture("bert", h, 768, 0, 768, L, 0);

  float* xa = A.alloc<float>(R * 640);
  float* xb = A.alloc<float>(R * 640);
  float* xp = A.alloc<float>(R * 2048);
  float* lo = A.alloc<float>(R * 512);
  {
    GemmPlanes gb;
    if (h_planes) { gb.in_hi = p768h; gb.in_lo = p768l; }
    gemm(L, L, h, 768, 768, W.benc_w, &W.t_benc, W.benc_b, 512, xa, 640, 0, ACT_NONE, 1, 0, nullptr, nullptr, ACT_NONE, 0.f,
         nullptr, 0, nullptr, 0, 1.f, &gb);
  }
  capture("d_en", xa, 640, 0, 512, L, 0);
  launch_bcast_cols(d_styles_, 256, 128, 128, xa, 640, 512, L.d_off, L.d_len, B, L.max_len, st);
  launch_bcast_cols(d_styles_, 256, 128, 128, xb, 640, 512, L.d_off, L.d_len, B, L.max_len, st);
  float* cur = xa; float* nxt = xb;
  for (int i = 0; i < 3; i++) {
    gemm(L, L, cur, 640, 640, W.dur_lstm[i].wih, &W.dur_lstm[i].t_ih, W.dur_lstm[i].bias, 2048, xp, 2048, 0);
    launch_lstm(xp, W.dur_lstm[i].whhT, lo, 512, 0, L.d_off, L.d_len, B, st, opt.precision != 0 && opt.lstm_fast_gates);
    LnArgs ln;
    ln.x = lo; ln.ldx = 512; ln.ada = r.sty_pro; ln.ada_ld = W.sty_pro_n; ln.ada_off = W.dur_ada[i];
    ln.eps = 1e-5f; ln.out = nxt; ln.ldo = 640; ln.ocol = 0; ln.off = L.d_off; ln.len = L.d_len;
    ln.B = B; ln.max_len = L.max_len; ln.C = 512;
    launch_layernorm(ln, st);
    std::swap(cur, nxt);
  }
  r.d = cur;
  capture("d", r.d, 640, 0, 640, L, 0);

  gemm(L, L, r.d, 640, 640, W.pred_lstm.wih, &W.pred_lstm.t_ih, W.pred_lstm.bias, 2048, xp, 2048, 0);
  launch_lstm(xp, W.pred_lstm.whhT, lo, 512, 0, L.d_off, L.d_len, B, st, opt.precision != 0 && opt.lstm_fast_gates);
  capture("dur_lstm", lo, 512, 0, 512, L, 0);
  float* logits = A.alloc<float>(R * 50);
  gemm(L, L, lo, 512, 512, W.durp_w, &W.t_durp, W.durp_b, 50, logits, 50, 0);
  capture("dur_logits", logits, 50, 0, 50, L, 0);
  r.pred_dur = A.alloc<int>(R);
  float* durf = A.alloc<float>(R);
  r.cum = A.alloc<int>((size_t)B * 512);
  r.total = A.alloc<int>(B);
  launch_duration(logits, 50, d_speeds_, r.pred_dur, durf, L.d_off, L.d_len, B, L.max_len, st);
  capture("dur_float", durf, 1, 0, 1, L, 0);
  for (auto& kv : inj_dur_) {
    const int b = kv.first;
    if (b >= B) throw ArgError("inject pred_dur: item index out of range");
    if ((int)kv.second.size() != L.len[b]) throw ArgError("inject pred_dur: length != n_tokens of the item");
    upload(r.pred_dur + L.off[b], kv.second.data(), kv.second.size() * sizeof(int));
  }
  launch_dur_scan(r.pred_dur, r.cum, 512, r.total, L.d_off, L.d_len, B, st);

  if (fork) join_lane1();
  else text_encoder();
  capture("t_en", r.t_en, 512, 0, 512, L, 0);

  set_lane_scratch(0, nullptr, nullptr, 0);
  set_lane_scratch(1, nullptr, nullptr, 0);
  KKX_CUDA(cudaMemcpyAsync(h_T_, r.total, B * sizeof(int), cudaMemcpyDeviceToHost, st));
  KKX_CUDA(cudaMemcpyAsync(h_pred_dur_, r.pred_dur, R * sizeof(int), cudaMemcpyDeviceToHost, st));
}

void Model::token_finish(Run& r) {
  const int B = B_;
  KKX_CUDA(cudaStreamSynchronize(stream_));
  r.T.resize(B);
  for (int b = 0; b < B; b++) {
    r.T[b] = h_T_[b];
    if (r.T[b] < 1 || r.T[b] > kMaxItemFrames)
      throw ArgError("item " + std::to_string(b) + ": " + std::to_string(r.T[b]) + " frames is outside 1.." +
                     std::to_string(kMaxItemFrames) + " (utterance too long for one call at this speed)");
  }
}

void Model::adain_blk(Run& r, Arena& A, const AdaBlkW& w, const float* x, int ldx, const Level& Lin,
                      const Level& Lout, const float* sty, int sld, float* out, int ldo, int ocol,
                      bool dry) {
  (void)r; (void)dry;
  cudaStream_t st = cur_;
  const int B = Lin.B;
  const int nch_in = (Lin.max_len + kStatRows - 1) / kStatRows;
  const int nch_out = (Lout.max_len + kStatRows - 1) / kStatRows;
  float* part = A.alloc<float>((size_t)B * std::max(nch_in, nch_out) * 2 * std::max(w.ci, w.co));
  float* sc1 = A.alloc<float>((size_t)B * w.ci);
  float* sh1 = A.alloc<float>((size_t)B * w.ci);
  float* sc2 = A.alloc<float>((size_t)B * w.co);
  float* sh2 = A.alloc<float>((size_t)B * w.co);
  float* t = A.alloc<float>((size_t)Lout.rows * w.co);

  launch_colstats(x, ldx, w.ci, part, Lin.d_off, Lin.d_len, B, Lin.max_len, st);
  launch_adain_coef(part, w.ci, Lin.max_len, Lin.d_len, sty, sld, w.sty1, 1e-5f, sc1, sh1, B, st);
  if (opt.precision == 1 && w.t1.w) {
    const int cpi = w.t1.Cpad, cpo = w.t2.Cpad;
    void* a1 = A.alloc_bytes((size_t)Lout.rows * cpi * 2);
    if (w.up)
      launch_pool_up_bf16(x, ldx, sc1, sh1, 0.2f, w.poolw, w.poolb, w.ci, a1, cpi, Lout.rows, Lin.d_off,
                          Lin.d_len, Lout.d_off, B, Lin.max_len, st);
    else
      launch_apply_bf16(x, ldx, w.ci, sc1, sh1, ACT_LRELU, 0.2f, nullptr, a1, cpi, Lin.rows, Lin.d_off,
                        Lin.d_len, B, Lin.max_len, st);
    tc_conv(A, a1, Lout.rows, w.t1, 1, 1, Lout, Lout, w.b1, t, w.co, 0, Lout, 1, 0, nullptr, 0, nullptr, 0, 1.f, false);
    launch_colstats(t, w.co, w.co, part, Lout.d_off, Lout.d_len, B, Lout.max_len, st);
    launch_adain_coef(part, w.co, Lout.max_len, Lout.d_len, sty, sld, w.sty2, 1e-5f, sc2, sh2, B, st);
    void* a2 = A.alloc_bytes((size_t)Lout.rows * cpo * 2);
    launch_apply_bf16(t, w.co, w.co, sc2, sh2, ACT_LRELU, 0.2f, nullptr, a2, cpo, Lout.rows, Lout.d_off,
                      Lout.d_len, B, Lout.max_len, st);
    const float* scp = x; int ldsc = ldx;
    if (w.w1x1) {
      void* a3 = A.alloc_bytes((size_t)Lin.rows * cpi * 2);
      float* s = A.alloc<float>((size_t)Lin.rows * w.co);
      launch_apply_bf16(x, ldx, w.ci, nullptr, nullptr, ACT_NONE, 0.f, nullptr, a3, cpi, Lin.rows, Lin.d_off,
                        Lin.d_len, B, Lin.max_len, st);
      tc_conv(A, a3, Lin.rows, w.t1x1, 1, 0, Lin, Lin, nullptr, s, w.co, 0, Lin, 1, 0, nullptr, 0, nullptr, 0, 1.f, false);
      scp = s; ldsc = w.co;
    }
    tc_conv(A, a2, Lout.rows, w.t2, 1, 1, Lout, Lout, w.b2, out, ldo, ocol, Lout, 1, 0, scp, ldsc, &Lin,
            w.up ? 1 : 0, 0.70710678118654752440f, false);
    return;
  }
  if (w.up) {
    float* p = A.alloc<float>((size_t)Lout.rows * w.ci);
    launch_pool_up(x, ldx, sc1, sh1, 0.2f, w.poolw, w.poolb, w.ci, p, w.ci, Lin.d_off, Lin.d_len,
                   Lout.d_off, B, Lin.max_len, st);
    gemm(Lout, Lout, p, w.ci, w.ci, w.w1, &w.s1, w.b1, w.co, t, w.co, 0, ACT_NONE, 3, 1);
  } else {
    gemm(Lin, Lin, x, ldx, w.ci, w.w1, &w.s1, w.b1, w.co, t, w.co, 0, ACT_NONE, 3, 1, sc1, sh1, ACT_LRELU, 0.2f);
  }
  launch_colstats(t, w.co, w.co, part, Lout.d_off, Lout.d_len, B, Lout.max_len, st);
  launch_adain_coef(part, w.co, Lout.max_len, Lout.d_len, sty, sld, w.sty2, 1e-5f, sc2, sh2, B, st);

  const float* sc = x; int ldsc = ldx;
  if (w.w1x1) {
    float* s = A.alloc<float>((size_t)Lin.rows * w.co);
    gemm(Lin, Lin, x, ldx, w.ci, w.w1x1, &w.s1x1, nullptr, w.co, s, w.co, 0);
    sc = s; ldsc = w.co;
  }
  gemm(Lout, Lout, t, w.co, w.co, w.w2, &w.s2, w.b2, w.co, out, ldo, ocol, ACT_NONE, 3, 1, sc2, sh2, ACT_LRELU, 0.2f,
       sc, ldsc, &Lin, w.up ? 1 : 0, 0.70710678118654752440f);
}

bool Model::use_stream_bf16(int C, int k, int B) const {
  return opt.precision == 1 && opt.stream_bf16 && arb_conv_supported(C, k, 5, B) && arb_tile_rows(C, k) == (C == 128 ? 256 : 128);
}

void Model::arb(Run& r, Arena& A, const ArbW& w, const float* x, const Level& L, const float* sty,
                int sld, float* xw, float* t1, float* out, float oscale, bool accumulate, const float* part_x,
                const void* x_bf16) {
  (void)r;
  cudaStream_t st = cur_;
  const int B = L.B, C = w.c, k = w.k;
  const int nch = (L.max_len + kStatRows - 1) / kStatRows;
  float* part = A.alloc<float>((size_t)B * nch * 2 * C);
  float* sc = A.alloc<float>((size_t)B * C);
  float* sh = A.alloc<float>((size_t)B * C);
  const int dil[3] = {1, 3, 5};
  const float* cur = x;
  const bool tc = opt.precision == 1;
  void* abuf = tc ? A.alloc_bytes((size_t)L.rows * w.t1[0].Cpad * 2) : nullptr;
  static const bool fused_ok = env_flag("KKX_ARB_FUSED", true);
  if (tc && fused_ok && arb_conv_supported(C, k, 5, B)) {
    ArbConvArgs base;
    base.C = C; base.ks = k; base.off = L.d_off; base.len = L.d_len; base.B = B; base.sum_m = L.sum_len;
    const int trows = arb_tile_rows(C, k);
    base.tile_start = trows == 512 ? L.d_tiles512 : trows == 256 ? L.d_tiles256 : L.d_tiles128;
    base.total_tiles = trows == 512 ? L.ntiles512 : trows == 256 ? L.ntiles256 : L.ntiles128;
    base.scale = sc; base.shift = sh; base.nchunk = nch;
    const bool sb = use_stream_bf16(C, k, B);
    void* xb0 = nullptr;
    if (sb && !x_bf16) xb0 = A.alloc_bytes((size_t)L.rows * C * 2);
    if (!part_x) launch_colstats(cur, C, C, part, L.d_off, L.d_len, B, L.max_len, st, xb0);
    else if (sb && !x_bf16) throw ArgError("arb: a bf16 stream with caller-provided statistics needs the bf16 input too");
    const void* curb = sb ? (x_bf16 ? x_bf16 : xb0) : nullptr;
    long long* tim = arb_timing_buf();
    static const int tim_ks = env_int("KKX_ARB_TIMING_KS", 0);
    if (tim_ks && tim_ks != k) tim = nullptr;
    for (int j = 0; j < 3; j++) {
      launch_adain_coef(j == 0 && part_x ? part_x : part, C, L.max_len, L.d_len, sty, sld, w.s1[j], 1e-5f, sc, sh, B, st);
      ArbConvArgs c1 = base;
      if (tim) c1.timing = tim + (C == 128 ? 0 : 64);
      c1.x = sb ? curb : (const void*)cur; c1.in_bf16 = sb ? 1 : 0; c1.alpha = w.a1[j]; c1.tmB = w.t1[j].tmap; c1.dil = dil[j];
      c1.pad = dil[j] * (k - 1) / 2; c1.bias = w.b1[j];
      c1.out_bf16 = static_cast<__nv_bfloat16*>(abuf); c1.part = part;
      launch_arb_conv(c1, st);
      launch_adain_coef(part, C, L.max_len, L.d_len, sty, sld, w.s2[j], 1e-5f, sc, sh, B, st);
      float* dst = (j == 2) ? out : xw;
      ArbConvArgs c2 = base;
      if (tim) c2.timing = tim + (C == 128 ? 32 : 96);
      c2.x = abuf; c2.in_bf16 = 1; c2.alpha = w.a2[j]; c2.tmB = w.t2[j].tmap; c2.dil = 1; c2.pad = (k - 1) / 2;
      c2.bias = w.b2[j];
      if (sb) {
        c2.res = static_cast<const float*>(curb); c2.res_bf16 = 1;
        if (j == 2) { c2.out_f32 = out; c2.oscale = oscale; c2.accumulate = accumulate ? 1 : 0; }
        else { c2.out_bf16 = reinterpret_cast<__nv_bfloat16*>(xw); c2.part = part; curb = xw; }
      } else {
        c2.out_f32 = dst; c2.res = cur;
        if (j == 2) { c2.oscale = oscale; c2.accumulate = accumulate ? 1 : 0; } else c2.part = part;
      }
      launch_arb_conv(c2, st);
      cur = dst;
    }
    return;
  }
  for (int j = 0; j < 3; j++) {
    launch_colstats(cur, C, C, part, L.d_off, L.d_len, B, L.max_len, st);
    launch_adain_coef(part, C, L.max_len, L.d_len, sty, sld, w.s1[j], 1e-5f, sc, sh, B, st);
    if (tc) {
      const int cp = w.t1[j].Cpad;
      launch_apply_bf16(cur, C, C, sc, sh, ACT_SNAKE, 0.f, w.a1[j], abuf, cp, L.rows, L.d_off, L.d_len, B, L.max_len, st);
      tc_conv(A, abuf, L.rows, w.t1[j], dil[j], dil[j] * (k - 1) / 2, L, L, w.b1[j], t1, C, 0, L, 1, 0, nullptr, 0,
              nullptr, 0, 1.f, false);
      launch_colstats(t1, C, C, part, L.d_off, L.d_len, B, L.max_len, st);
      launch_adain_coef(part, C, L.max_len, L.d_len, sty, sld, w.s2[j], 1e-5f, sc, sh, B, st);
      launch_apply_bf16(t1, C, C, sc, sh, ACT_SNAKE, 0.f, w.a2[j], abuf, cp, L.rows, L.d_off, L.d_len, B, L.max_len, st);
      float* dst = (j == 2) ? out : xw;
      tc_conv(A, abuf, L.rows, w.t2[j], 1, (k - 1) / 2, L, L, w.b2[j], dst, C, 0, L, 1, 0, cur, C, &L, 0,
              j == 2 ? oscale : 1.f, j == 2 && accumulate);
      cur = dst;
      continue;
    }
    ConvArgs c1 = gemm_args(L, cur, C, C, w.w1[j], w.b1[j], C, t1, C, 0);
    c1.ks = k; c1.dil = dil[j]; c1.pad = dil[j] * (k - 1) / 2;
    c1.pscale = sc; c1.pshift = sh; c1.pld = C; c1.pact = ACT_SNAKE; c1.palpha = w.a1[j];
    launch_conv_f32(c1, st);
    launch_colstats(t1, C, C, part, L.d_off, L.d_len, B, L.max_len, st);
    launch_adain_coef(part, C, L.max_len, L.d_len, sty, sld, w.s2[j], 1e-5f, sc, sh, B, st);
    float* dst = (j == 2) ? out : xw;
    ConvArgs c2 = gemm_args(L, t1, C, C, w.w2[j], w.b2[j], C, dst, C, 0);
    c2.ks = k; c2.dil = 1; c2.pad = (k - 1) / 2;
    c2.pscale = sc; c2.pshift = sh; c2.pld = C; c2.pact = ACT_SNAKE; c2.palpha = w.a2[j];
    c2.res = cur; c2.ldr = C; c2.res_off = L.d_off;
    if (j == 2) { c2.oscale = oscale; c2.accumulate = accumulate ? 1 : 0; }
    launch_conv_f32(c2, st);
    cur = dst;
  }
}

void Model::frame_phase(Run& r, int b0, int b1, bool dry) {
  use_lane(0);
  cudaStream_t st = stream_;
  Arena& A = frA_;
  const int B = b1 - b0;
  const bool fork = !dry && can_fork(B);
  cudaStream_t st1 = fork ? stream2_ : stream_;
  std::vector<int> T(r.T.begin() + b0, r.T.begin() + b1), T2(B), T20(B), T120(B), one(B, 1);
  long long maxS = 0;
  for (int b = 0; b < B; b++) {
    T2[b] = 2 * T[b]; T20[b] = 20 * T[b]; T120[b] = 120 * T[b] + 1;
    maxS = std::max(maxS, 600LL * T[b]);
  }
  Level FR = make_level(T, A), FR2 = make_level(T2, A), G20 = make_level(T20, A), G120 = make_level(T120, A);
  const int* tok_off = tokL_.d_off + b0;
  const int* tok_len = tokL_.d_len + b0;
  const int* cum = r.cum + (size_t)b0 * 512;
  const float* sty_pro = r.sty_pro + (size_t)b0 * W.sty_pro_n;
  const float* sty_dec = r.sty_dec + (size_t)b0 * W.sty_dec_n;
  std::vector<int> ph_off(B);
  std::vector<long long> s_loc(B), s_glob(B);
  {
    int po = 0; long long so = 0;
    for (int b = 0; b < B; b++) {
      ph_off[b] = po; po += 9 * T2[b];
      s_loc[b] = so; so += 600LL * T[b];
      s_glob[b] = sample_off_[b0 + b];
    }
  }
  int* d_ph_off = A.alloc<int>(B);
  long long* d_s_loc = A.alloc<long long>(B);
  long long* d_s_glob = A.alloc<long long>(B);
  upload(d_ph_off, ph_off.data(), B * sizeof(int));
  upload(d_s_loc, s_loc.data(), B * sizeof(long long));
  upload(d_s_glob, s_glob.data(), B * sizeof(long long));
  float* wav24 = nullptr;
  long long* d_s_len = nullptr;
  long long max_out = 0;
  if (resample_) {
    std::vector<long long> s_len(B);
    for (int b = 0; b < B; b++) {
      s_len[b] = 600LL * T[b];
      max_out = std::max(max_out, (s_len[b] * rs_U_ + rs_D_ - 1) / rs_D_);
    }
    wav24 = A.alloc<float>((size_t)(s_loc[B - 1] + s_len[B - 1]));
    d_s_len = A.alloc<long long>(B);
    upload(d_s_len, s_len.data(), B * sizeof(long long));
  }

  int* idx = A.alloc<int>(FR.rows);
  float* en = A.alloc<float>((size_t)FR.rows * 640);
  float* x514 = A.alloc<float>((size_t)FR.rows * 520);
  launch_expand_idx(cum, 512, tok_len, idx, FR.d_off, FR.d_len, B, FR.max_len, st);
  launch_gather_rows(r.d, 640, tok_off, idx, FR.d_off, FR.d_len, 640, en, 640, 0, B, FR.max_len, st);
  launch_gather_rows(r.t_en, 512, tok_off, idx, FR.d_off, FR.d_len, 512, x514, 520, 0, B, FR.max_len, st);
  if (debug_ && !dry) {
    bool any = false;
    for (int b = 0; b < B; b++) any = any || want_debug(b0 + b);
    if (any) {
      KKX_CUDA(cudaStreamSynchronize(st));
      std::vector<int> hi(FR.rows);
      KKX_CUDA(cudaMemcpy(hi.data(), idx, FR.rows * sizeof(int), cudaMemcpyDeviceToHost));
      for (int b = 0; b < B; b++) {
        if (!want_debug(b0 + b)) continue;
        DebugStage s; s.rows = FR.len[b]; s.cols = 1; s.data.resize(FR.len[b]);
        for (int j = 0; j < FR.len[b]; j++) s.data[j] = (float)hi[FR.off[b] + j];
        dbg_["idx#" + std::to_string(b0 + b)] = std::move(s);
      }
    }
  }
  capture("en", en, 640, 0, 640, FR, b0);
  capture("asr", x514, 520, 0, 512, FR, b0);

  float* xp = A.alloc<float>((size_t)FR.rows * 2048);
  float* shd = A.alloc<float>((size_t)FR.rows * 512);
  {
    const size_t cap = std::max((size_t)FR.rows * 640, (size_t)FR2.rows * 512);
    float* hi = A.alloc<float>(cap); float* lo = A.alloc<float>(cap);
    set_lane_scratch(0, hi, lo, cap);
    float* hi1 = A.alloc<float>(cap); float* lo1 = A.alloc<float>(cap);
    set_lane_scratch(1, hi1, lo1, cap);
  }
  gemm(FR, FR, en, 640, 640, W.shared_lstm.wih, &W.shared_lstm.t_ih, W.shared_lstm.bias, 2048, xp, 2048, 0);
  launch_lstm(xp, W.shared_lstm.whhT, shd, 512, 0, FR.d_off, FR.d_len, B, st, opt.precision != 0 && opt.lstm_fast_gates);
  capture("shared_lstm", shd, 512, 0, 512, FR, b0);
  float* curves[2];
  if (fork) fork_lane1();
  for (int k = 0; k < 2; k++) {
    const AdaBlkW* blk = k == 0 ? W.f0blk : W.nblk;
    if (fork) use_lane(k);
    float* y0 = A.alloc<float>((size_t)FR.rows * 512);
    float* y1 = A.alloc<float>((size_t)FR2.rows * 256);
    float* y2 = A.alloc<float>((size_t)FR2.rows * 256);
    adain_blk(r, A, blk[0], shd, 512, FR, FR, sty_pro, W.sty_pro_n, y0, 512, 0, dry);
    adain_blk(r, A, blk[1], y0, 512, FR, FR2, sty_pro, W.sty_pro_n, y1, 256, 0, dry);
    adain_blk(r, A, blk[2], y1, 256, FR2, FR2, sty_pro, W.sty_pro_n, y2, 256, 0, dry);
    curves[k] = A.alloc<float>(FR2.rows);
    launch_conv_f32(gemm_args(FR2, y2, 256, 256, k == 0 ? W.f0proj_w : W.nproj_w,
                              k == 0 ? W.f0proj_b : W.nproj_b, 1, curves[k], 1, 0), cur_);
  }
  use_lane(0);
  if (fork) join_lane1();
  float* f0 = curves[0]; float* nc = curves[1];
  set_lane_scratch(0, nullptr, nullptr, 0);
  set_lane_scratch(1, nullptr, nullptr, 0);
  if (!dry) {
    for (int k = 0; k < 2; k++) {
      for (auto& kv : (k == 0 ? inj_f0_ : inj_n_)) {
        const int b = kv.first - b0;
        if (kv.first >= B_) throw ArgError("inject F0/N: item index out of range");
        if (b < 0 || b >= B) continue;
        if ((int)kv.second.size() != FR2.len[b]) throw ArgError("inject F0/N: length != 2T of the item");
        upload((k == 0 ? f0 : nc) + FR2.off[b], kv.second.data(), kv.second.size() * sizeof(float));
      }
    }
  }
  capture("F0", f0, 1, 0, 1, FR2, b0);
  capture("N", nc, 1, 0, 1, FR2, b0);

  if (fork) { fork_lane1(); use_lane(1); }
  float* phase = A.alloc<float>((size_t)9 * FR2.sum_len + 16);
  float* src = A.alloc<float>((size_t)600 * FR.sum_len + 16);
  float* har = A.alloc<float>((size_t)G120.rows * 24);
  launch_sine_phase(f0, FR2.d_off, FR2.d_len, phase, d_ph_off, B, st1);
  if (!dry && d_noise_) {
    for (int b = 0; b < B; b++)
      if (600LL * T[b] * 9 > noise_n_) throw ArgError("noise buffer smaller than 600*T*9");
  }
  launch_sine_source(f0, FR2.d_off, FR2.d_len, phase, d_ph_off, d_noise_, opt.noise_seed, W.lin_w,
                     W.lin_b, src, d_s_loc, B, maxS, st1);
  if (debug_ && !dry) {
    bool any = false;
    for (int b = 0; b < B; b++) any = any || want_debug(b0 + b);
    if (any) KKX_CUDA(cudaStreamSynchronize(st1));
    for (int b = 0; b < B; b++) {
      if (!want_debug(b0 + b)) continue;
      DebugStage s; s.rows = 600LL * T[b]; s.cols = 1; s.data.resize(s.rows);
      KKX_CUDA(cudaMemcpy(s.data.data(), src + s_loc[b], s.rows * sizeof(float), cudaMemcpyDeviceToHost));
      dbg_["har_source#" + std::to_string(b0 + b)] = std::move(s);
    }
  }
  launch_stft(src, d_s_loc, har, 24, G120.d_off, G120.d_len, opt.stft_replicate, B, G120.max_len, st1);
  capture("har", har, 24, 0, 22, G120, b0);

  const size_t n20 = (size_t)G20.rows * 256, n120 = (size_t)G120.rows * 128;
  float* xs0 = A.alloc<float>(n20);
  float* x0 = A.alloc<float>(n20);
  float* w0 = A.alloc<float>(n20);
  float* t0 = A.alloc<float>(n20);
  float* acc0 = A.alloc<float>(n20);
  if (opt.precision == 1) {
    void* col = A.alloc_bytes((size_t)G20.rows * W.t_nc0.Cpad * 2);
    launch_im2col_bf16(har, 24, 22, 12, 6, 3, col, W.t_nc0.Cpad, G20.rows, G120.d_off, G120.d_len, G20.d_off,
                       G20.d_len, B, G20.max_len, st1);
    tc_conv(A, col, G20.rows, W.t_nc0, 1, 0, G20, G20, W.nc0_b, xs0, 256, 0, G20, 1, 0, nullptr, 0, nullptr, 0, 1.f, false);
  } else {
    ConvArgs c = gemm_args(G20, har, 24, 22, W.nc0_w, W.nc0_b, 256, xs0, 256, 0);
    c.in_off = G120.d_off; c.in_len = G120.d_len;
    c.ks = 12; c.stride = 6; c.pad = 3;
    launch_conv_f32(c, st1);
  }
  arb(r, A, W.nres[0], xs0, G20, sty_dec, W.sty_dec_n, w0, t0, xs0, 1.f, false);
  capture("gen.x_source.0", xs0, 256, 0, 256, G20, b0);
  float* xs1 = A.alloc<float>(n120);
  float* x1 = A.alloc<float>(n120);
  float* w1 = A.alloc<float>(n120);
  float* t1 = A.alloc<float>(n120);
  float* acc1 = A.alloc<float>(n120);
  float* pxs1 = nullptr;
  if (opt.precision == 1 && opt.fuse_noise_stats && !use_stream_bf16(128, W.nres[1].k, B)) {
    pxs1 = A.alloc<float>((size_t)B * ((G120.max_len + kStatRows - 1) / kStatRows) * 2 * 128);
    launch_pointwise_conv_stats(har, 24, 22, W.nc1_w, W.nc1_b, xs1, 128, pxs1, G120.d_off, G120.d_len, B, G120.max_len,
                                G120.sum_len, st1);
  } else if (opt.precision == 1) {
    void* hb = A.alloc_bytes((size_t)G120.rows * W.t_nc1.Cpad * 2);
    launch_apply_bf16(har, 24, 22, nullptr, nullptr, ACT_NONE, 0.f, nullptr, hb, W.t_nc1.Cpad, G120.rows, G120.d_off,
                      G120.d_len, B, G120.max_len, st1);
    tc_conv(A, hb, G120.rows, W.t_nc1, 1, 0, G120, G120, W.nc1_b, xs1, 128, 0, G120, 1, 0, nullptr, 0, nullptr, 0, 1.f, false);
  } else {
    launch_conv_f32(gemm_args(G120, har, 24, 22, W.nc1_w, W.nc1_b, 128, xs1, 128, 0), st1);
  }
  arb(r, A, W.nres[1], xs1, G120, sty_dec, W.sty_dec_n, w1, t1, xs1, 1.f, false, pxs1);
  capture("gen.x_source.1", xs1, 128, 0, 128, G120, b0);
  use_lane(0);

  float* xA = A.alloc<float>((size_t)FR.rows * 1096);
  float* xB = A.alloc<float>((size_t)FR.rows * 1096);
  launch_curve_conv(f0, FR2.d_off, FR2.d_len, W.f0conv_w, W.f0conv_b, x514, 520, 512, FR.d_off, FR.d_len, B, FR.max_len, st);
  launch_curve_conv(nc, FR2.d_off, FR2.d_len, W.nconv_w, W.nconv_b, x514, 520, 513, FR.d_off, FR.d_len, B, FR.max_len, st);
  adain_blk(r, A, W.enc, x514, 520, FR, FR, sty_dec, W.sty_dec_n, xA, 1096, 0, dry);
  capture("dec.encode", xA, 1096, 0, 1024, FR, b0);
  launch_conv_f32(gemm_args(FR, x514, 520, 512, W.asr_w, W.asr_b, 64, xA, 1096, 1024), st);
  launch_copy_cols(x514, 520, 512, xA, 1096, 1088, 2, FR.d_off, FR.d_len, B, FR.max_len, st);
  launch_copy_cols(xA, 1096, 1024, xB, 1096, 1024, 66, FR.d_off, FR.d_len, B, FR.max_len, st);
  float* dcur = xA; float* dnxt = xB;
  for (int i = 0; i < 3; i++) {
    adain_blk(r, A, W.dec[i], dcur, 1096, FR, FR, sty_dec, W.sty_dec_n, dnxt, 1096, 0, dry);
    std::swap(dcur, dnxt);
    capture(("dec.decode." + std::to_string(i)).c_str(), dcur, 1096, 0, 1024, FR, b0);
  }
  float* y = A.alloc<float>((size_t)FR2.rows * 512);
  adain_blk(r, A, W.dec[3], dcur, 1096, FR, FR2, sty_dec, W.sty_dec_n, y, 512, 0, dry);
  capture("dec.decode.3", y, 512, 0, 512, FR2, b0);

  void* ybf = nullptr;
  if (opt.precision == 1) {
    ybf = A.alloc_bytes((size_t)FR2.rows * 512 * 2);
    launch_apply_bf16(y, 512, 512, nullptr, nullptr, ACT_LRELU, 0.1f, nullptr, ybf, 512, FR2.rows, FR2.d_off,
                      FR2.d_len, B, FR2.max_len, st);
  }
  if (opt.precision == 1 && opt.fuse_phases && !dry) {
    alignas(64) unsigned char tmA[128];
    make_tmap_bf16(tmA, ybf, W.tups0_all.Cpad, FR2.rows, W.tups0_all.Cpad, 128);
    TcConvArgs a;
    a.tmA = tmA; a.tmB = W.tups0_all.tmap;
    a.Cpad = W.tups0_all.Cpad; a.Ci = W.tups0_all.Ci; a.Co = 256; a.ks = 2; a.dil = -1;
    a.in_off = FR2.d_off; a.m_len = FR2.d_len; a.max_m = FR2.max_len; a.B = B; a.sum_m = FR2.sum_len;
    a.bias = W.ups0_b; a.out = x0; a.ldo = 256; a.ocol = 0; a.out_off = G20.d_off; a.ors = 10;
    a.nphase = 10;
    for (int ph = 0; ph < 10; ph++) { const int q0 = ph < 5 ? 1 : 0; a.phase_pad[ph] = -q0; a.phase_oro[ph] = q0 * 10 + ph - 5; }
    if (opt.conv_pair && W.tups0_all.pair_map(256)) {
      a.tmB_c = W.tups0_all.pair_map(256); a.pair = 1; a.tile_start = FR2.d_tiles128; a.ntiles_m = FR2.ntiles128;
    }
    launch_conv_tc(a, st);
  } else
  for (int ph = 0; ph < 10; ph++) {
    const int q0 = ph < 5 ? 1 : 0;
    if (opt.precision == 1) {
      tc_conv(A, ybf, FR2.rows, W.tups0[ph], -1, -q0, FR2, FR2, W.ups0_b, x0, 256, 0, G20, 10, q0 * 10 + ph - 5,
              nullptr, 0, nullptr, 0, 1.f, false);
      continue;
    }
    ConvArgs c = gemm_args(FR2, y, 512, 512, W.ups0[ph], W.ups0_b, 256, x0, 256, 0);
    c.out_off = G20.d_off;
    c.ks = 2; c.dil = -1; c.pad = -q0; c.stride = 1;
    c.ors = 10; c.oro = q0 * 10 + ph - 5;
    c.pact = ACT_LRELU; c.pslope = 0.1f;
    launch_conv_f32(c, st);
  }
  if (fork) join_lane1();
  capture("gen.ups.0", x0, 256, 0, 256, G20, b0);
  {
    float* px = nullptr;
    void* xb = nullptr;
    if (opt.precision == 1) {
      px = A.alloc<float>((size_t)B * ((G20.max_len + kStatRows - 1) / kStatRows) * 2 * 256);
      const bool sb0 = use_stream_bf16(256, 3, B) && use_stream_bf16(256, 7, B) && use_stream_bf16(256, 11, B);
      xb = sb0 ? A.alloc_bytes((size_t)G20.rows * 256 * 2) : nullptr;
      launch_add_rows_stats(x0, xs0, x0, 256, px, G20.d_off, G20.d_len, B, G20.max_len, st, xb);
    } else {
      launch_add_rows(x0, xs0, x0, 256, G20.d_off, G20.d_len, B, G20.max_len, st);
    }
    for (int j = 0; j < 3; j++)
      arb(r, A, W.res[j], x0, G20, sty_dec, W.sty_dec_n, w0, t0, acc0, 1.0f / 3.0f, j > 0, px, xb);
  }
// ... 83 lines not shown
```

kokorox_b200/csrc/testapi.cu:

```cuda
#include "../../include/kkx_test.h"
#include "kernels.h"
#include "model.h"
#include <algorithm>
#include <cstring>
#include <limits>
#include <string>
#include <vector>

using namespace kkx;
static thread_local std::string t_err;

namespace {
struct DevBuf {
  void* p = nullptr;
  DevBuf(const void* host, size_t bytes) {
    KKX_CUDA(cudaMalloc(&p, bytes ? bytes : 4));
    if (host && bytes) KKX_CUDA(cudaMemcpy(p, host, bytes, cudaMemcpyHostToDevice));
  }
  ~DevBuf() { if (p) cudaFree(p); }
  template <class T> T* as() { return static_cast<T*>(p); }
};
template <class F> int run(int device, F&& f) {
  try {
    int n = 0;
// ... 146 lines not shown
    DevBuf dx(xin.data(), xin.size() * 4), dw(hw.data(), hw.size() * 2), db(bias, bias ? Co * 4 : 0);
    DevBuf dps(pscale, pscale ? Ci * 4 : 0), dph(pshift, pshift ? Ci * 4 : 0), dal(palpha, palpha ? Ci * 4 : 0);
    DevBuf dres(res, res ? (size_t)res_rows * Co * 4 : 0), dout(out, (size_t)out_rows * Co * 4);
    DevBuf dab(nullptr, (size_t)rows_total * Cpad * 2);
    KKX_CUDA(cudaMemset(dab.p, 0xFF, (size_t)rows_total * Cpad * 2));
    int meta[5] = {off, L, m_len, 0, 0};
    DevBuf dm(meta, sizeof meta);
    launch_apply_bf16(dx.as<float>(), Ci, Ci, pscale ? dps.as<float>() : nullptr, pshift ? dph.as<float>() : nullptr,
                      pact, pslope, palpha ? dal.as<float>() : nullptr, dab.p, Cpad, rows_total, dm.as<int>(),
                      dm.as<int>() + 1, 1, L, 0);
    alignas(64) unsigned char tmA[128], tmB[128];
    make_tmap_bf16(tmA, dab.p, Cpad, rows_total, Cpad, 128);
    make_tmap_bf16(tmB, dw.p, (long long)ks * Cpad, Co, (long long)ks * Cpad, tc_box_n(Co));
    TcConvArgs a;
    a.tmA = tmA; a.tmB = tmB; a.Cpad = Cpad; a.Ci = Ci; a.Co = Co; a.ks = ks; a.dil = dil; a.pad = pad;
    a.in_off = dm.as<int>(); a.m_len = dm.as<int>() + 2; a.max_m = m_len; a.B = 1; a.sum_m = m_len;
    a.bias = bias ? db.as<float>() : nullptr;
    a.out = dout.as<float>(); a.ldo = Co; a.ocol = 0; a.out_off = dm.as<int>() + 3; a.ors = ors; a.oro = oro;
    a.res = res ? dres.as<float>() : nullptr; a.ldr = Co; a.rcol = 0; a.res_off = dm.as<int>() + 4;
    a.res_shift = res_shift; a.oscale = oscale; a.accumulate = accumulate;
    launch_conv_tc(a, 0);
    KKX_CUDA(cudaDeviceSynchronize());
    KKX_CUDA(cudaMemcpy(out, dout.p, (size_t)out_rows * Co * 4, cudaMemcpyDeviceToHost));
  });
}

static inline float host_tf32(float f) {
  uint32_t u; memcpy(&u, &f, 4);
  u = (u + 0x1000u) & ~0x1FFFu;
  float r; memcpy(&r, &u, 4);
  return r;
}

KKX_API int kkx_test_conv_tf32(int device, const float* x, int L, int Ci, const float* w, const float* bias,
                               int Co, int ks, int dil, int pad, int nprod, int eact, float* out) {
  return run(device, [&] {
    const int Cpad = (Ci + 63) & ~63;
    const int off = kGapRows, rows_total = (off + L + kGapRows + 7) & ~7;
    std::vector<float> whi((size_t)Co * ks * Cpad, 0.f), wlo((size_t)Co * ks * Cpad, 0.f);
    for (int o = 0; o < Co; o++)
      for (int k = 0; k < ks; k++)
        for (int c = 0; c < Ci; c++) {
          const float f = w[((size_t)o * ks + k) * Ci + c];
          const float hi = host_tf32(f);
          whi[((size_t)o * ks + k) * Cpad + c] = hi;
          wlo[((size_t)o * ks + k) * Cpad + c] = host_tf32(f - hi);
        }
    std::vector<float> xin((size_t)rows_total * Ci, 0.f);
    memcpy(xin.data() + (size_t)off * Ci, x, (size_t)L * Ci * 4);
    DevBuf dx(xin.data(), xin.size() * 4), dwh(whi.data(), whi.size() * 4), dwl(wlo.data(), wlo.size() * 4);
    DevBuf db(bias, bias ? Co * 4 : 0), dout(nullptr, (size_t)L * Co * 4);
    DevBuf dah(nullptr, (size_t)rows_total * Cpad * 4), dal(nullptr, (size_t)rows_total * Cpad * 4);
    KKX_CUDA(cudaMemset(dah.p, 0xFF, (size_t)rows_total * Cpad * 4));
    KKX_CUDA(cudaMemset(dal.p, 0xFF, (size_t)rows_total * Cpad * 4));
    int meta[4] = {off, L, 0, 0};
    DevBuf dm(meta, sizeof meta);
    launch_apply_tf32(dx.as<float>(), Ci, Ci, nullptr, nullptr, ACT_NONE, 0.f, dah.as<float>(), dal.as<float>(), Cpad,
                      rows_total, dm.as<int>(), dm.as<int>() + 1, 1, L, 0);
    alignas(64) unsigned char tA[128], tA2[128], tB[128], tB2[128];
    make_tmap_f32(tA, dah.p, Cpad, rows_total, Cpad, 128);
    make_tmap_f32(tA2, dal.p, Cpad, rows_total, Cpad, 128);
    make_tmap_f32(tB, dwh.p, (long long)ks * Cpad, Co, (long long)ks * Cpad, tc_box_n_tf32(Co));
    make_tmap_f32(tB2, dwl.p, (long long)ks * Cpad, Co, (long long)ks * Cpad, tc_box_n_tf32(Co));
    TcConvArgs a;
    a.tmA = tA; a.tmA2 = tA2; a.tmB = tB; a.tmB2 = tB2; a.tf32 = 1; a.nprod = nprod; a.eact = eact;
    a.Cpad = Cpad; a.Ci = Ci; a.Co = Co; a.ks = ks; a.dil = dil; a.pad = pad;
    a.in_off = dm.as<int>(); a.m_len = dm.as<int>() + 1; a.max_m = L; a.B = 1; a.sum_m = L;
    a.bias = bias ? db.as<float>() : nullptr;
    a.out = dout.as<float>(); a.ldo = Co; a.ocol = 0; a.out_off = dm.as<int>() + 2; a.ors = 1; a.oro = 0;
    launch_conv_tc(a, 0);
    KKX_CUDA(cudaDeviceSynchronize());
    KKX_CUDA(cudaMemcpy(out, dout.p, (size_t)L * Co * 4, cudaMemcpyDeviceToHost));
  });
}

static int conv_f16x3_impl(int device, const float* x, int L, int Ci, const float* w, const float* bias,
                           int Co, int ks, int dil, int pad, int eact, int kernel, const float* res, float oscale, float* out) {
  return run(device, [&] {
    const int Cpad = (Ci + 63) & ~63;
    const int off = kGapRows, rows_total = (off + L + kGapRows + 7) & ~7;
    std::vector<float> wp((size_t)Co * ks * Cpad, 0.f);
    for (int o = 0; o < Co; o++)
      for (int k = 0; k < ks; k++)
        for (int c = 0; c < Ci; c++) wp[((size_t)o * ks + k) * Cpad + c] = w[((size_t)o * ks + k) * Ci + c];
    std::vector<unsigned short> whi(wp.size()), wlo(wp.size());
    const float wscale = split_f16_host(wp.data(), wp.size(), whi.data(), wlo.data());
    std::vector<float> xin((size_t)rows_total * Ci, 0.f);
    memcpy(xin.data() + (size_t)off * Ci, x, (size_t)L * Ci * 4);
    DevBuf dx(xin.data(), xin.size() * 4), dwh(whi.data(), whi.size() * 2), dwl(wlo.data(), wlo.size() * 2);
    DevBuf db(bias, bias ? Co * 4 : 0), dout(nullptr, (size_t)L * Co * 4);
    DevBuf dah(nullptr, (size_t)rows_total * Cpad * 2), dal(nullptr, (size_t)rows_total * Cpad * 2);
    KKX_CUDA(cudaMemset(dah.p, 0xFF, (size_t)rows_total * Cpad * 2));
    KKX_CUDA(cudaMemset(dal.p, 0xFF, (size_t)rows_total * Cpad * 2));
    int meta[4] = {off, L, 0, 0};
    DevBuf dm(meta, sizeof meta);
    launch_apply_f16x2(dx.as<float>(), Ci, Ci, nullptr, nullptr, ACT_NONE, 0.f, dah.p, dal.p, Cpad,
                       rows_total, dm.as<int>(), dm.as<int>() + 1, 1, L, 0);
    alignas(64) unsigned char tA[128], tA2[128], tB[128], tB2[128], tBc[128], tB2c[128];
    make_tmap_f16(tA, dah.p, Cpad, rows_total, Cpad, 128);
    make_tmap_f16(tA2, dal.p, Cpad, rows_total, Cpad, 128);
    make_tmap_f16(tB, dwh.p, (long long)ks * Cpad, Co, (long long)ks * Cpad, tc_box_n_tf32(Co));
    make_tmap_f16(tB2, dwl.p, (long long)ks * Cpad, Co, (long long)ks * Cpad, tc_box_n_tf32(Co));
    const int nt = (L + 127) / 128;
    int tiles[2] = {0, nt};
    DevBuf dt(tiles, sizeof tiles);
    TcConvArgs a;
    a.tmA = tA; a.tmA2 = tA2; a.tmB = tB; a.tmB2 = tB2; a.tf32 = 1; a.nprod = 3; a.eact = eact;
    a.f16 = 1; a.wscale = wscale / kSplitF16Scale;
    if (tc_box_n_tf32(Co) == 128) {
      make_tmap_f16(tBc, dwh.p, (long long)ks * Cpad, Co, (long long)ks * Cpad, 64);
      make_tmap_f16(tB2c, dwl.p, (long long)ks * Cpad, Co, (long long)ks * Cpad, 64);
      a.tmB_c = tBc; a.tmB2_c = tB2c;
    }
    a.Cpad = Cpad; a.Ci = Ci; a.Co = Co; a.ks = ks; a.dil = dil; a.pad = pad;
    a.in_off = dm.as<int>(); a.m_len = dm.as<int>() + 1; a.max_m = L; a.B = 1; a.sum_m = L;
    a.bias = bias ? db.as<float>() : nullptr;
    a.out = dout.as<float>(); a.ldo = Co; a.ocol = 0; a.out_off = dm.as<int>() + 2; a.ors = 1; a.oro = 0;
    a.tile_start = dt.as<int>(); a.ntiles_m = nt;
    DevBuf dres(res, res ? (size_t)L * Co * 4 : 0);
    if (res) { a.res = dres.as<float>(); a.ldr = Co; a.rcol = 0; a.res_off = dm.as<int>() + 2; a.res_shift = 0; }
    a.oscale = oscale;
    if (kernel) a.force_kernel = 1;
    if (kernel == 1) { a.tile_start = nullptr; a.ntiles_m = 0; }
    a.pair = (kernel == 0 || kernel == 3) ? 1 : 0;
    launch_conv_tc(a, 0);
    KKX_CUDA(cudaDeviceSynchronize());
    KKX_CUDA(cudaMemcpy(out, dout.p, (size_t)L * Co * 4, cudaMemcpyDeviceToHost));
  });
}

KKX_API int kkx_test_conv_f16x3(int device, const float* x, int L, int Ci, const float* w, const float* bias,
                                int Co, int ks, int dil, int pad, int eact, float* out) {
  return conv_f16x3_impl(device, x, L, Ci, w, bias, Co, ks, dil, pad, eact, 0, nullptr, 1.f, out);
}

KKX_API int kkx_test_conv_f16x3_k(int device, const float* x, int L, int Ci, const float* w, const float* bias,
                                  int Co, int ks, int dil, int pad, int eact, int kernel, const float* res, float oscale,
                                  float* out) {
  return conv_f16x3_impl(device, x, L, Ci, w, bias, Co, ks, dil, pad, eact, kernel, res, oscale, out);
}

KKX_API int kkx_test_lstm(int device, const float* xproj, const float* whhT, int N, float* out) {
  return run(device, [&] {
    DevBuf dx(xproj, (size_t)N * 2048 * 4), dw(whhT, (size_t)2 * 256 * 1024 * 4), dout(nullptr, (size_t)N * 512 * 4);
    int meta[2] = {0, N};
    DevBuf dm(meta, sizeof meta);
    launch_lstm(dx.as<float>(), dw.as<float>(), dout.as<float>(), 512, 0, dm.as<int>(), dm.as<int>() + 1, 1, 0);
    KKX_CUDA(cudaDeviceSynchronize());
    KKX_CUDA(cudaMemcpy(out, dout.p, (size_t)N * 512 * 4, cudaMemcpyDeviceToHost));
  });
}

KKX_API int kkx_test_lstm_batch(int device, const float* xproj, const float* whhT, int B, const int* off,
                                const int* len, int rows, float* out) {
  return run(device, [&] {
    DevBuf dx(xproj, (size_t)rows * 2048 * 4), dw(whhT, (size_t)2 * 256 * 1024 * 4), dout(out, (size_t)rows * 512 * 4);
    DevBuf doff(off, B * 4), dlen(len, B * 4);
    launch_lstm(dx.as<float>(), dw.as<float>(), dout.as<float>(), 512, 0, doff.as<int>(), dlen.as<int>(), B, 0);
    KKX_CUDA(cudaDeviceSynchronize());
    KKX_CUDA(cudaMemcpy(out, dout.p, (size_t)rows * 512 * 4, cudaMemcpyDeviceToHost));
  });
}

KKX_API int kkx_test_lstm_batch_v(int device, const float* xproj, const float* whhT, int B, const int* off,
                                  const int* len, int rows, int variant, int reps, float* out, float* ms) {
  return run(device, [&] {
    DevBuf dx(xproj, (size_t)rows * 2048 * 4), dw(whhT, (size_t)2 * 256 * 1024 * 4), dout(out, (size_t)rows * 512 * 4);
    DevBuf doff(off, B * 4), dlen(len, B * 4);
    cudaEvent_t e0, e1;
    KKX_CUDA(cudaEventCreate(&e0)); KKX_CUDA(cudaEventCreate(&e1));
    launch_lstm(dx.as<float>(), dw.as<float>(), dout.as<float>(), 512, 0, doff.as<int>(), dlen.as<int>(), B, 0, variant);
    KKX_CUDA(cudaEventRecord(e0, 0));
    for (int i = 0; i < reps; i++)
      launch_lstm(dx.as<float>(), dw.as<float>(), dout.as<float>(), 512, 0, doff.as<int>(), dlen.as<int>(), B, 0, variant);
    KKX_CUDA(cudaEventRecord(e1, 0));
    KKX_CUDA(cudaDeviceSynchronize());
    float t = 0.f;
    KKX_CUDA(cudaEventElapsedTime(&t, e0, e1));
    if (ms) *ms = reps > 0 ? t / reps : 0.f;
    cudaEventDestroy(e0); cudaEventDestroy(e1);
    KKX_CUDA(cudaMemcpy(out, dout.p, (size_t)rows * 512 * 4, cudaMemcpyDeviceToHost));
  });
}

KKX_API int kkx_test_pointwise_conv_stats(int device, const float* x, const float* w, const float* bias, int B,
                                          const int* off, const int* len, int rows, int max_len, float* out, float* part,
                                          float* part_ref) {
  return run(device, [&] {
    const int nchunk = (max_len + kStatRows - 1) / kStatRows;
    const size_t np = (size_t)B * nchunk * 2 * 128;
    DevBuf dx(x, (size_t)rows * 24 * 4), dw(w, (size_t)22 * 128 * 4), db(bias, 128 * 4), dout(out, (size_t)rows * 128 * 4);
    DevBuf dp(part, np * 4), dpr(part_ref, np * 4), doff(off, B * 4), dlen(len, B * 4);
    long long sum_m = 0;
    for (int b = 0; b < B; b++) sum_m += len[b];
    launch_pointwise_conv_stats(dx.as<float>(), 24, 22, dw.as<float>(), db.as<float>(), dout.as<float>(), 128, dp.as<float>(),
                                doff.as<int>(), dlen.as<int>(), B, max_len, sum_m, 0);
    launch_colstats(dout.as<float>(), 128, 128, dpr.as<float>(), doff.as<int>(), dlen.as<int>(), B, max_len, 0);
    KKX_CUDA(cudaDeviceSynchronize());
    KKX_CUDA(cudaMemcpy(out, dout.p, (size_t)rows * 128 * 4, cudaMemcpyDeviceToHost));
    KKX_CUDA(cudaMemcpy(part, dp.p, np * 4, cudaMemcpyDeviceToHost));
    KKX_CUDA(cudaMemcpy(part_ref, dpr.p, np * 4, cudaMemcpyDeviceToHost));
  });
}

KKX_API int kkx_test_layernorm(int device, const float* x, const float* res, const float* w, const float* b,
                               const float* ada, int rows, int C, float eps, float slope, float* out,
                               unsigned short* pl_hi, unsigned short* pl_lo) {
  return run(device, [&] {
    const size_t n = (size_t)rows * C;
    DevBuf dx(x, n * 4), dr(res, res ? n * 4 : 0), dw(w, w ? (size_t)C * 4 : 0), db(b, b ? (size_t)C * 4 : 0);
    DevBuf da(ada, ada ? (size_t)2 * C * 4 : 0), dout(nullptr, n * 4), dhi(nullptr, pl_hi ? n * 2 : 0), dlo(nullptr, pl_lo ? n * 2 : 0);
    int meta[2] = {0, rows};
    DevBuf dm(meta, sizeof meta);
    LnArgs a;
    a.x = dx.as<float>(); a.ldx = C;
    if (res) { a.res = dr.as<float>(); a.ldr = C; }
    if (w) { a.w = dw.as<float>(); a.b = db.as<float>(); }
    if (ada) { a.ada = da.as<float>(); a.ada_ld = 2 * C; a.ada_off = 0; }
    a.eps = eps; a.slope = slope; a.out = dout.as<float>(); a.ldo = C; a.ocol = 0;
    a.off = dm.as<int>(); a.len = dm.as<int>() + 1; a.B = 1; a.max_len = rows; a.C = C;
    if (pl_hi) { a.pl_hi = dhi.p; a.pl_lo = dlo.p; a.pl_ld = C; }
    launch_layernorm(a, 0);
    KKX_CUDA(cudaDeviceSynchronize());
    KKX_CUDA(cudaMemcpy(out, dout.p, n * 4, cudaMemcpyDeviceToHost));
    if (pl_hi) {
      KKX_CUDA(cudaMemcpy(pl_hi, dhi.p, n * 2, cudaMemcpyDeviceToHost));
      KKX_CUDA(cudaMemcpy(pl_lo, dlo.p, n * 2, cudaMemcpyDeviceToHost));
    }
  });
}

KKX_API int kkx_test_im2col(int device, const float* in, int rows_in, int B, const int* in_off, const int* in_len,
                            const int* out_off, const int* out_len, int rows_out, int max_out_len, int Cpad, int generic,
                            unsigned short* out) {
  return run(device, [&] {
    DevBuf di(in, (size_t)rows_in * 24 * 4), dout(out, (size_t)rows_out * Cpad * 2);
    DevBuf dio(in_off, B * 4), dil(in_len, B * 4), doo(out_off, B * 4), dol(out_len, B * 4);
    launch_im2col_bf16(di.as<float>(), 24, 22, 12, 6, 3, dout.p, Cpad, rows_out, dio.as<int>(), dil.as<int>(), doo.as<int>(),
                       dol.as<int>(), B, max_out_len, 0, generic);
    KKX_CUDA(cudaDeviceSynchronize());
    KKX_CUDA(cudaMemcpy(out, dout.p, (size_t)rows_out * Cpad * 2, cudaMemcpyDeviceToHost));
  });
}

KKX_API int kkx_test_attention(int device, const float* qkv, int N, float* ctx) {
  return run(device, [&] {
    DevBuf dq(qkv, (size_t)N * 2304 * 4), dout(nullptr, (size_t)N * 768 * 4);
    int meta[2] = {0, N};
    DevBuf dm(meta, sizeof meta);
    launch_attention(dq.as<float>(), dout.as<float>(), dm.as<int>(), dm.as<int>() + 1, 1, N, 0);
    KKX_CUDA(cudaDeviceSynchronize());
    KKX_CUDA(cudaMemcpy(ctx, dout.p, (size_t)N * 768 * 4, cudaMemcpyDeviceToHost));
  });
}

KKX_API int kkx_test_attention_batch(int device, const float* qkv, int B, const int* off, const int* len, int rows,
                                     int umma, float* ctx) {
  return run(device, [&] {
    int max_len = 0;
    for (int b = 0; b < B; b++) max_len = std::max(max_len, len[b]);
    DevBuf dq(qkv, (size_t)rows * 2304 * 4), dout(ctx, (size_t)rows * 768 * 4);
    DevBuf doff(off, (size_t)B * 4), dlen(len, (size_t)B * 4);
    if (umma) {
      const size_t nf = attention_umma_scratch_floats(rows, B);
      DevBuf ds(nullptr, nf * 4);
      KKX_CUDA(cudaMemset(ds.p, 0xFF, nf * 4));
      launch_attention_umma(dq.as<float>(), ds.as<float>(), dout.as<float>(), doff.as<int>(), dlen.as<int>(), B, max_len, rows, 0);
      KKX_CUDA(cudaDeviceSynchronize());
    } else {
      launch_attention(dq.as<float>(), dout.as<float>(), doff.as<int>(), dlen.as<int>(), B, max_len, 0);
      KKX_CUDA(cudaDeviceSynchronize());
    }
    KKX_CUDA(cudaMemcpy(ctx, dout.p, (size_t)rows * 768 * 4, cudaMemcpyDeviceToHost));
  });
}

KKX_API int kkx_test_adain_coef(int device, const float* x, int L, int C, const float* gamma_beta,
                                float* scale, float* shift) {
  return run(device, [&] {
    const int nch = (L + kStatRows - 1) / kStatRows;
    DevBuf dx(x, (size_t)L * C * 4), dgb(gamma_beta, (size_t)2 * C * 4), dpart(nullptr, (size_t)nch * 2 * C * 4);
    DevBuf dsc(nullptr, C * 4), dsh(nullptr, C * 4);
    int meta[2] = {0, L};
    DevBuf dm(meta, sizeof meta);
    launch_colstats(dx.as<float>(), C, C, dpart.as<float>(), dm.as<int>(), dm.as<int>() + 1, 1, L, 0);
    launch_adain_coef(dpart.as<float>(), C, L, dm.as<int>() + 1, dgb.as<float>(), 2 * C, 0, 1e-5f,
                      dsc.as<float>(), dsh.as<float>(), 1, 0);
    KKX_CUDA(cudaDeviceSynchronize());
    KKX_CUDA(cudaMemcpy(scale, dsc.p, C * 4, cudaMemcpyDeviceToHost));
    KKX_CUDA(cudaMemcpy(shift, dsh.p, C * 4, cudaMemcpyDeviceToHost));
  });
}

static inline uint16_t host_bf16(float f) {
  uint32_t u; memcpy(&u, &f, 4);
  return (uint16_t)((u + 0x7FFFu + ((u >> 16) & 1u)) >> 16);
}

}

static int arb_conv_test(int device, const float* x, int B, const int* lens, int C, int in_bf16,
                         const float* scale, const float* shift, const float* alpha, const float* w,
                         const float* bias, int ks, int dil, const float* res, int res_bf16, float oscale,
                         int accumulate, int want_bf16, float* out, float* sums, int desc_mode) {
  return run(device, [&] {
    if (!arb_conv_supported(C, ks, dil, B)) throw ArgError("kkx_test_arb_conv: unsupported shape");
    std::vector<int> off(B), tiles(B + 1, 0);
    const int MT = arb_tile_rows(C, ks);
    int o = kGapRows, maxL = 0; long long sumL = 0;
    for (int b = 0; b < B; b++) {
      off[b] = o; o = (o + lens[b] + kGapRows + 7) & ~7;
      tiles[b + 1] = tiles[b] + (lens[b] + MT - 1) / MT;
      maxL = std::max(maxL, lens[b]); sumL += lens[b];
    }
    const int rows = o;
    const float qnan = std::numeric_limits<float>::quiet_NaN();
    std::vector<float> hx((size_t)rows * C, qnan), hres((size_t)rows * C, qnan), hout((size_t)rows * C, qnan);
    size_t src = 0;
    for (int b = 0; b < B; b++) {
      memcpy(hx.data() + (size_t)off[b] * C, x + src * C, (size_t)lens[b] * C * 4);
      if (res) memcpy(hres.data() + (size_t)off[b] * C, res + src * C, (size_t)lens[b] * C * 4);
      memcpy(hout.data() + (size_t)off[b] * C, out + src * C, (size_t)lens[b] * C * 4);
      src += lens[b];
    }
    std::vector<uint16_t> hxb;
    if (in_bf16) { hxb.resize(hx.size()); for (size_t i = 0; i < hx.size(); i++) hxb[i] = host_bf16(hx[i]); }
    std::vector<uint16_t> hw((size_t)C * ks * C);
    for (size_t i = 0; i < hw.size(); i++) hw[i] = host_bf16(w[i]);
    DevBuf dx(in_bf16 ? (const void*)hxb.data() : (const void*)hx.data(), hx.size() * (in_bf16 ? 2 : 4));
    DevBuf dw(hw.data(), hw.size() * 2), db(bias, C * 4), dsc(scale, (size_t)B * C * 4), dsh(shift, (size_t)B * C * 4);
    std::vector<uint16_t> hresb;
    if (res && res_bf16) { hresb.resize(hres.size()); for (size_t i = 0; i < hres.size(); i++) hresb[i] = host_bf16(hres[i]); }
    DevBuf dal(alpha, C * 4), dres(res ? (res_bf16 ? (const void*)hresb.data() : (const void*)hres.data()) : nullptr,
                                   res ? hres.size() * (res_bf16 ? 2 : 4) : 0);
    DevBuf dout(hout.data(), hout.size() * 4), doutb(nullptr, hout.size() * 2);
    KKX_CUDA(cudaMemset(doutb.p, 0xFF, hout.size() * 2));
    const int nchunk = (maxL + 127) / 128;
    DevBuf dpart(nullptr, (size_t)B * nchunk * 2 * C * 4);
    KKX_CUDA(cudaMemset(dpart.p, 0, (size_t)B * nchunk * 2 * C * 4));
    DevBuf doff(off.data(), B * 4), dlen(lens, B * 4), dts(tiles.data(), (B + 1) * 4);
    alignas(64) unsigned char tmB[128];
    make_tmap_bf16(tmB, dw.p, (long long)ks * C, C, (long long)ks * C, tc_box_n(C));
    ArbConvArgs a;
    a.x = dx.p; a.in_bf16 = in_bf16; a.scale = dsc.as<float>(); a.shift = dsh.as<float>(); a.alpha = dal.as<float>();
    a.tmB = tmB; a.C = C; a.ks = ks; a.dil = dil; a.pad = dil * (ks - 1) / 2;
    a.off = doff.as<int>(); a.len = dlen.as<int>(); a.tile_start = dts.as<int>(); a.B = B; a.total_tiles = tiles[B];
    a.sum_m = sumL; a.bias = db.as<float>();
    a.out_bf16 = want_bf16 ? doutb.as<__nv_bfloat16>() : nullptr;
    a.out_f32 = want_bf16 ? nullptr : dout.as<float>();
    a.res = res ? dres.as<float>() : nullptr; a.res_bf16 = res ? res_bf16 : 0; a.oscale = oscale; a.accumulate = accumulate;
    a.part = sums ? dpart.as<float>() : nullptr; a.nchunk = nchunk; (void)desc_mode;
    launch_arb_conv(a, 0);
    KKX_CUDA(cudaDeviceSynchronize());
    if (want_bf16) {
      std::vector<uint16_t> hb(hout.size());
      KKX_CUDA(cudaMemcpy(hb.data(), doutb.p, hb.size() * 2, cudaMemcpyDeviceToHost));
      for (size_t i = 0; i < hb.size(); i++) { uint32_t u = (uint32_t)hb[i] << 16; memcpy(&hout[i], &u, 4); }
    } else {
      KKX_CUDA(cudaMemcpy(hout.data(), dout.p, hout.size() * 4, cudaMemcpyDeviceToHost));
    }
    src = 0;
    for (int b = 0; b < B; b++) {
      memcpy(out + src * C, hout.data() + (size_t)off[b] * C, (size_t)lens[b] * C * 4);
      src += lens[b];
    }
    if (sums) {
      std::vector<float> hp((size_t)B * nchunk * 2 * C);
      KKX_CUDA(cudaMemcpy(hp.data(), dpart.p, hp.size() * 4, cudaMemcpyDeviceToHost));
      for (int b = 0; b < B; b++)
        for (int k = 0; k < 2; k++)
          for (int c = 0; c < C; c++) {
            double acc = 0.0;
            for (int ch = 0; ch < (lens[b] + 127) / 128; ch++) acc += hp[(((size_t)b * nchunk + ch) * 2 + k) * C + c];
            sums[((size_t)b * 2 + k) * C + c] = (float)acc;
          }
    }
  });
}

extern "C" {

KKX_API int kkx_test_arb_conv(int device, const float* x, int B, const int* lens, int C, int in_bf16,
                              const float* scale, const float* shift, const float* alpha, const float* w,
                              const float* bias, int ks, int dil, const float* res, float oscale,
                              int accumulate, int want_bf16, float* out, float* sums, int desc_mode) {
  return arb_conv_test(device, x, B, lens, C, in_bf16, scale, shift, alpha, w, bias, ks, dil, res, 0, oscale, accumulate,
                       want_bf16, out, sums, desc_mode);
}

KKX_API int kkx_test_arb_conv_stream(int device, const float* x, int B, const int* lens, int C, const float* scale,
                                     const float* shift, const float* alpha, const float* w, const float* bias, int ks,
                                     int dil, const float* res, float oscale, int accumulate, int want_bf16, float* out,
                                     float* sums) {
  return arb_conv_test(device, x, B, lens, C, 1, scale, shift, alpha, w, bias, ks, dil, res, 1, oscale, accumulate,
                       want_bf16, out, sums, 0);
}

}
```

Measured before the change: 10690.

## Add CTA-pair (cta_group::2) path for C=256 arbitrary-kernel convolutions

Adds a two-CTA cluster variant of the arbitrary-kernel conv for C=256. Each CTA of the pair loads half of the weight tile via multicast TMA, and the leader CTA issues 256-row pair UMMAs over both CTAs' row tiles, with barriers signalled across the cluster. It is selected for large kernel sizes when there are enough tiles to fill half the SMs. Separately, the default C=256 fp32-input conv1 path now uses the balanced-producer variant, controlled by an env flag. The pair path adds cluster synchronisation and tail handling for odd tile counts.

```diff
diff --git a/kokorox_b200/csrc/capi.cu b/kokorox_b200/csrc/capi.cu
--- a/kokorox_b200/csrc/capi.cu
+++ b/kokorox_b200/csrc/capi.cu
@@ -771,6 +771,7 @@
     else if (k == "gemm_pair") o.gemm_pair = value ? 1 : 0;
     else if (k == "fuse_planes") o.fuse_planes = value ? 1 : 0;
     else if (k == "conv_pair") o.conv_pair = value ? 1 : 0;
+    else if (k == "arb_pair") o.arb_pair = value ? 1 : 0;
     else if (k == "fork_max_batch") { if (value < 0 || value > 512) throw ArgError("fork_max_batch must be in 0..512"); o.fork_max_batch = (int)value; }
     else if (k == "max_tokens") { if (value < 512) throw ArgError("max_tokens must be >= 512"); ctx->max_tokens = value; }
     else if (k == "coalesce") {
diff --git a/kokorox_b200/csrc/kernels.h b/kokorox_b200/csrc/kernels.h
--- a/kokorox_b200/csrc/kernels.h
+++ b/kokorox_b200/csrc/kernels.h
@@ -90,6 +90,7 @@
   const float* scale = nullptr; const float* shift = nullptr;
   const float* alpha = nullptr;
   const void* tmB = nullptr;
+  const void* tmB_pair = nullptr; int pair = 0;
   int C = 0, ks = 1, dil = 1, pad = 0;
   const int* off = nullptr; const int* len = nullptr;
   const int* tile_start = nullptr;
diff --git a/kokorox_b200/csrc/kernels_arb.cu b/kokorox_b200/csrc/kernels_arb.cu
--- a/kokorox_b200/csrc/kernels_arb.cu
+++ b/kokorox_b200/csrc/kernels_arb.cu
@@ -26,14 +26,14 @@
 constexpr int kArbThreads = 512;
 constexpr int kArbMaxB = 512;
 
-template <int BN, int MSUB, bool T>
+template <int BN, int MSUB, bool T, bool PAIR = false>
 struct ArbCfg {
   static constexpr int KCH = BN / 64;
   static constexpr int RA = MSUB * 128 + 56;
   static constexpr uint32_t A_SLOT = RA * 128;
   static constexpr int NA = (BN == 128 && (!T || MSUB == 4)) ? 2 : 3;
-  static constexpr uint32_t B_STAGE = BN * 128;
-  static constexpr int NB = (T && MSUB == 4) ? 4 : (BN == 128) ? 6 : 3;
+  static constexpr uint32_t B_STAGE = (PAIR ? BN / 2 : BN) * 128;
+  static constexpr int NB = PAIR ? 6 : (T && MSUB == 4) ? 4 : (BN == 128) ? 6 : 3;
   static constexpr int PITCH = 36;
   static constexpr uint32_t STG = T ? 0 : 2 * 128 * PITCH * 4;
   static constexpr uint32_t STAT = 4 * BN * 2 * 4;
@@ -49,25 +49,31 @@
 }
 
 struct TileCur {
-  int b, mt;
+  int b, mt, t;
   __device__ __forceinline__ void init(const int* ts, int B, int tile) {
     int lo = 0, hi = B;
     while (hi - lo > 1) {
       const int mid = (lo + hi) >> 1;
       if (ts[mid] <= tile) lo = mid; else hi = mid;
     }
-    b = lo; mt = tile - ts[lo];
+    b = lo; mt = tile - ts[lo]; t = tile;
   }
   __device__ __forceinline__ void next(const int* ts) {
-    mt++;
+    mt++; t++;
     while (ts[b] + mt >= ts[b + 1]) { b++; mt = 0; if (ts[b] < 0) break; }
   }
+  template <bool PAIR> __device__ __forceinline__ void step(const int* ts, int last) {
+    if (!PAIR) { next(ts); return; }
+    if (t < last) next(ts);
+    if (t < last) next(ts);
+  }
 };
 
-template <int BN, int MSUB, bool CONV2, bool T, bool POST = false, int SB = 0, bool PB = false>
+template <int BN, int MSUB, bool CONV2, bool T, bool POST = false, int SB = 0, bool PB = false, bool PAIR = false>
 __global__ void __launch_bounds__(kArbThreads, 1) arb_conv_kernel(const __grid_constant__ CUtensorMap tmB, ArbConvArgs a) {
   static_assert(SB == 0 || (!POST && (CONV2 || SB == 1)), "stream-bf16 variants: conv1 SB=1, conv2 SB=1 (bf16 out) / SB=2 (fp32 out)");
-  static_assert(!PB || (T && !CONV2 && !POST && SB == 0 && MSUB == 2), "balanced-producer variant: conv1, transposed accumulator, fp32 input");
+  static_assert(!PB || (!CONV2 && !POST && SB == 0 && (T ? MSUB == 2 : MSUB == 1)), "balanced-producer variant: conv1, fp32 input");
+  static_assert(!PAIR || (BN == 256 && MSUB == 1 && !T && !POST && SB == 0 && !PB), "CTA pairs: C = 256, rows as M, fp32 stream");
   constexpr bool XIN_BF = CONV2 || SB != 0;
   constexpr bool OUT_BF = !CONV2 || SB == 1;
   static_assert(!T || (BN == 128 && (MSUB == 2 || MSUB == 4)), "transposed mode: C = 128, 256- or 512-row tiles");
@@ -77,9 +83,10 @@
   constexpr int NPW = PB ? 8 : 14 - NEW;
   constexpr int kProdThreads = NPW * 32;
   constexpr int kProdRows = kProdThreads / 8;
-  using Cfg = ArbCfg<BN, MSUB, T>;
+  using Cfg = ArbCfg<BN, MSUB, T, PAIR>;
   constexpr int KCH = Cfg::KCH, NA = Cfg::NA, NB = Cfg::NB, PITCH = Cfg::PITCH;
   constexpr int MT = MSUB * 128;
+  constexpr uint32_t NCTA = PAIR ? 2 : 1;
   extern __shared__ uint8_t smem_raw[];
   const uint32_t base = (smem_u32(smem_raw) + 1023u) & ~1023u;
   uint8_t* const gbase = smem_raw + (base - smem_u32(smem_raw));
@@ -103,6 +110,7 @@
 
   const int warp = threadIdx.x >> 5, lane = threadIdx.x & 31;
   const int B = a.B;
+  const uint32_t rank = PAIR ? cluster_ctarank() : 0u;
 #pragma unroll 1
   for (int i = threadIdx.x; i <= B + 1; i += kArbThreads) s_ts[i] = i <= B ? a.tile_start[i] : -1;
 #pragma unroll 1
@@ -110,24 +118,36 @@
 
   if (warp == 0 && lane == 0) {
     asm volatile("prefetch.tensormap [%0];" ::"l"(&tmB) : "memory");
-    for (int s = 0; s < NA; s++) { mbar_init(fullA(s), kProdThreads / 32); mbar_init(emptyA(s), 1); }
+    for (int s = 0; s < NA; s++) { mbar_init(fullA(s), NCTA * (kProdThreads / 32)); mbar_init(emptyA(s), 1); }
     for (int s = 0; s < NB; s++) { mbar_init(fullB(s), 1); mbar_init(emptyB(s), 1); }
-    for (int j = 0; j < 2; j++) { mbar_init(tfull(j), 1); mbar_init(tempty(j), NEW); }
+    for (int j = 0; j < 2; j++) { mbar_init(tfull(j), 1); mbar_init(tempty(j), NCTA * NEW); }
     asm volatile("fence.mbarrier_init.release.cluster;" ::: "memory");
     asm volatile("fence.proxy.async.shared::cta;" ::: "memory");
   }
   if (warp == 1) {
-    asm volatile("tcgen05.alloc.cta_group::1.sync.aligned.shared::cta.b32 [%0], %1;" ::"r"(tmem_slot), "r"(512u) : "memory");
-    asm volatile("tcgen05.relinquish_alloc_permit.cta_group::1.sync.aligned;" ::: "memory");
+    if (PAIR) {
+      asm volatile("tcgen05.alloc.cta_group::2.sync.aligned.shared::cta.b32 [%0], %1;" ::"r"(tmem_slot), "r"(512u) : "memory");
+      asm volatile("tcgen05.relinquish_alloc_permit.cta_group::2.sync.aligned;" ::: "memory");
+    } else {
+      asm volatile("tcgen05.alloc.cta_group::1.sync.aligned.shared::cta.b32 [%0], %1;" ::"r"(tmem_slot), "r"(512u) : "memory");
+      asm volatile("tcgen05.relinquish_alloc_permit.cta_group::1.sync.aligned;" ::: "memory");
+    }
   }
   tc_fence_before();
-  __syncthreads();
+  if (PAIR) cluster_sync_all();
+  else __syncthreads();
   tc_fence_after();
   uint32_t tmem_base;
   asm volatile("ld.shared.b32 %0, [%1];" : "=r"(tmem_base) : "r"(tmem_slot) : "memory");
 
-  const int t_begin = (int)(((long long)a.total_tiles * blockIdx.x) / gridDim.x);
-  const int t_end = (int)(((long long)a.total_tiles * (blockIdx.x + 1)) / gridDim.x);
+  const int t_last = a.total_tiles - 1;
+  const int nunits = PAIR ? (a.total_tiles + 1) >> 1 : a.total_tiles;
+  const int nworkers = PAIR ? (int)(gridDim.x >> 1) : (int)gridDim.x;
+  const int worker = PAIR ? (int)(blockIdx.x >> 1) : (int)blockIdx.x;
+  const int t_begin = (int)(((long long)nunits * worker) / nworkers);
+  const int t_end = (int)(((long long)nunits * (worker + 1)) / nworkers);
+  const int tile0 = PAIR ? min(2 * t_begin + (int)rank, t_last) : t_begin;
+  auto unit_valid = [&](int u) { return !PAIR || 2 * u + (int)rank <= t_last; };
   const int ks = a.ks, dil = a.dil, pad = a.pad;
 
   if (warp == 0) {
@@ -144,19 +164,25 @@
             const int s = g % NB;
             mbar_wait(emptyB(s), (((uint32_t)(g / NB)) & 1u) ^ 1u);
             TICK(0);
-            mbar_expect_tx(fullB(s), Cfg::B_STAGE);
-            tma_load_2d(b_base + s * Cfg::B_STAGE, &tmB, tap * BN + c * 64, 0, fullB(s));
+            if (PAIR) {
+              const uint32_t lead_full = mapa_u32(fullB(s), 0);
+              if (rank == 0) mbar_expect_tx(fullB(s), 2 * Cfg::B_STAGE);
+              tma_load_2d_pair(b_base + s * Cfg::B_STAGE, &tmB, tap * BN + c * 64, (int)rank * (BN / 2), lead_full);
+            } else {
+              mbar_expect_tx(fullB(s), Cfg::B_STAGE);
+              tma_load_2d(b_base + s * Cfg::B_STAGE, &tmB, tap * BN + c * 64, 0, fullB(s));
+            }
             TICK(1);
           }
       }
       TIM_FLUSH(0, 2);
     }
   } else if (warp == 1) {
-    if (lane == 0 && t_begin < t_end) {
-      constexpr uint32_t idesc = umma_idesc_bf16(128, BN);
+    if (lane == 0 && t_begin < t_end && rank == 0) {
+      constexpr uint32_t idesc = umma_idesc_bf16(PAIR ? 256 : 128, BN);
       int gA = 0, gB = 0, ti = 0;
       TileCur cur;
-      cur.init(s_ts, B, t_begin);
+      cur.init(s_ts, B, tile0);
       const bool resident = KCH * ks <= NB;
       TIM_DECL(4);
 #pragma unroll 1
@@ -201,17 +227,19 @@
                 const uint64_t ad = umma_desc_sw128(slot + (uint32_t)(sub * 128 + tap * dil) * 128u);
                 const uint32_t td = tmem_base + (uint32_t)((buf * MSUB + sub) * BN);
 #pragma unroll
-                for (int k = 0; k < 4; k++)
-                  umma_bf16(td, ad + (uint64_t)(2 * k), bd + (uint64_t)(2 * k), idesc, (c | tap | k) ? 1u : 0u);
+                for (int k = 0; k < 4; k++) {
+                  if (PAIR) umma_f16_pair(td, ad + (uint64_t)(2 * k), bd + (uint64_t)(2 * k), idesc, (c | tap | k) ? 1u : 0u);
+                  else umma_bf16(td, ad + (uint64_t)(2 * k), bd + (uint64_t)(2 * k), idesc, (c | tap | k) ? 1u : 0u);
+                }
               }
             }
-            if (!resident) umma_commit(emptyB(sb));
+            if (!resident) { if (PAIR) umma_commit_pair(emptyB(sb)); else umma_commit(emptyB(sb)); }
             TICK(3);
           }
-          umma_commit(emptyA(sa));
-        }
-        umma_commit(tfull(buf));
-        cur.next(s_ts);
+          if (PAIR) umma_commit_pair(emptyA(sa)); else umma_commit(emptyA(sa));
+        }
+        if (PAIR) umma_commit_pair(tfull(buf)); else umma_commit(tfull(buf));
+        cur.step<PAIR>(s_ts, t_last);
       }
       TIM_FLUSH(4, 4);
     }
@@ -346,7 +374,8 @@
       TICK(7);
     }
     TIM_FLUSH(8, 9);
-  } else if (!T && warp < 10) {
+  } else if (!T && warp < 2 + NEW) {
+    constexpr int NG = NEW / 4;
     const int eg = (warp - 2) >> 2;
     const int q = warp & 3;
     const int et = q * 32 + lane;
@@ -358,7 +387,7 @@
     float* const stat_f = reinterpret_cast<float*>(gbase + (stat_base - base));
     const float* const st_rd = buf_f + tr * PITCH + c4;
     float* const st_wr = buf_f + et * PITCH;
-    constexpr int NCH = BN / 64;
+    constexpr int NCH = BN / (32 * NG);
     constexpr int RS = 16 * BN;
     const float2 os2 = make_float2(a.oscale, a.oscale);
     const bool accum = a.accumulate != 0;
@@ -368,7 +397,7 @@
       const int row = m0 + sub * 128 + tr;
       const int left = L - row;
       if (SB) {
-        const __nv_bfloat16* rp = reinterpret_cast<const __nv_bfloat16*>(a.res) + (size_t)(off + row) * BN + ((2 * ci + eg) * 32 + c4);
+        const __nv_bfloat16* rp = reinterpret_cast<const __nv_bfloat16*>(a.res) + (size_t)(off + row) * BN + ((NG * ci + eg) * 32 + c4);
 #pragma unroll
         for (int i = 0; i < 8; i++)
           if (16 * i < left) {
@@ -377,7 +406,7 @@
                                 __uint_as_float(w.y << 16), __uint_as_float(w.y & 0xFFFF0000u));
           }
       } else {
-        const float* rp = a.res + (size_t)(off + row) * BN + ((2 * ci + eg) * 32 + c4);
+        const float* rp = a.res + (size_t)(off + row) * BN + ((NG * ci + eg) * 32 + c4);
 #pragma unroll
         for (int i = 0; i < 8; i++)
           if (16 * i < left) rv[i] = *reinterpret_cast<const float4*>(rp + i * RS);
@@ -390,21 +419,33 @@
     long long tim_acc[9] = {0}; long long tim_last = clock64();
     const bool tim_on = a.timing && blockIdx.x == 0 && warp == 2 && lane == 0;
 #endif
-    if (t_begin < t_end) {
-      cur.init(s_ts, B, t_begin);
+    auto release_acc = [&](int buf) {
+      tc_fence_before();
+      if (lane == 0) {
+        if (PAIR) mbar_arrive_cluster(mapa_u32(tempty(buf), 0));
+        else asm volatile("mbarrier.arrive.shared::cta.b64 _, [%0];" ::"r"(tempty(buf)) : "memory");
+      }
+    };
+    if (t_begin < t_end && unit_valid(t_begin)) {
+      cur.init(s_ts, B, tile0);
       fetch(s_len[cur.b], s_off[cur.b], cur.mt * MT, 0, rv0);
       fetch(s_len[cur.b], s_off[cur.b], cur.mt * MT, 1, rv1);
     }
 #pragma unroll 1
     for (int tile = t_begin; tile < t_end; tile++, ti++) {
+      const int buf = ti & 1;
+      if (PAIR && !unit_valid(tile)) {
+        mbar_wait(tfull(buf), ((uint32_t)(ti >> 1)) & 1u);
+        release_acc(buf);
+        break;
+      }
       const int b = cur.b;
       const int L = s_len[b], off = s_off[b];
       const int m0 = cur.mt * MT;
       const int nsub = min(MSUB, (L - m0 + 127) >> 7);
       const int E = nsub * NCH;
-      const int buf = ti & 1;
-      cur.next(s_ts);
-      const bool has_next = tile + 1 < t_end;
+      cur.step<PAIR>(s_ts, t_last);
+      const bool has_next = tile + 1 < t_end && unit_valid(tile + 1);
       const int nL = has_next ? s_len[cur.b] : 0, noff = has_next ? s_off[cur.b] : 0, nm0 = cur.mt * MT;
       TICK(8);
       mbar_wait(tfull(buf), ((uint32_t)(ti >> 1)) & 1u);
@@ -414,14 +455,11 @@
         constexpr bool FULL = decltype(full_tag)::value;
         const int sub = e / NCH, ci = e & (NCH - 1);
         const int row = m0 + sub * 128 + tr;
-        const int n = (2 * ci + eg) * 32 + c4;
+        const int n = (NG * ci + eg) * 32 + c4;
         {
           uint32_t v[32];
           tmem_ld32(tmem_base + ((uint32_t)(q * 32) << 16) + (uint32_t)((buf * MSUB + sub) * BN + n - c4), v);
-          if (e == E - 1) {
-            tc_fence_before();
-            if (lane == 0) asm volatile("mbarrier.arrive.shared::cta.b64 _, [%0];" ::"r"(tempty(buf)) : "memory");
-          }
+          if (e == E - 1) release_acc(buf);
           TICK(1);
           asm volatile("bar.sync %0, 128;" ::"r"(bar_id) : "memory");
           TICK(2);
@@ -483,8 +521,9 @@
           }
           if (ci == NCH - 1) {
             asm volatile("bar.sync %0, 128;" ::"r"(bar_id) : "memory");
-            if (t < BN / 2) {
-              const int nn = ((t >> 5) * 2 + eg) * 32 + (t & 31);
+#pragma unroll
+            for (int c = t; c < BN / NG; c += 128) {
+              const int nn = ((c >> 5) * NG + eg) * 32 + (c & 31);
               float* pp = a.part + ((size_t)b * a.nchunk + (size_t)((m0 >> 7) + sub)) * 2 * BN + nn;
               const float* sf = stat_f + 2 * nn;
               pp[0] = (sf[0] + sf[2 * BN]) + (sf[4 * BN] + sf[6 * BN]);
@@ -524,9 +563,10 @@
     constexpr int XE = XIN_BF ? 2 : 4;
     const uint32_t sw = (uint32_t)rl * 128u + (uint32_t)((cg ^ (rl & 7)) << 4);
 
+    const uint32_t fullA_lead = PAIR ? mapa_u32(fullA(0), 0) : 0u;
     TileCur lc; int l_c = 0, l_g = 0;
     TileCur sc_; int s_c = 0, s_g = 0, gA = 0, coef_b = -1;
-    if (F > 0) { lc.init(s_ts, B, t_begin); sc_ = lc; }
+    if (F > 0) { lc.init(s_ts, B, tile0); sc_ = lc; }
     float2 cA[4], cB[4], cI[4];
 #ifdef KKX_ARB_TIMING
     long long tim_acc[5] = {0}; long long tim_last = clock64();
@@ -552,7 +592,7 @@
           }
         }
       }
-      if (++l_g == ngc) { l_g = 0; if (++l_c == KCH) { l_c = 0; lc.next(s_ts); } }
+      if (++l_g == ngc) { l_g = 0; if (++l_c == KCH) { l_c = 0; lc.step<PAIR>(s_ts, t_last); } }
     };
     auto process = [&](Raw (&rb)[GP][RPP]) {
       const int b = sc_.b;
@@ -622,9 +662,12 @@
       if (++s_g == ngc) {
         asm volatile("fence.proxy.async.shared::cta;" ::: "memory");
         __syncwarp();
-        if (lane == 0) asm volatile("mbarrier.arrive.shared::cta.b64 _, [%0];" ::"r"(fullA(sa)) : "memory");
+        if (lane == 0) {
+          if (PAIR) mbar_arrive_cluster(fullA_lead + (uint32_t)sa * 8u);
+          else asm volatile("mbarrier.arrive.shared::cta.b64 _, [%0];" ::"r"(fullA(sa)) : "memory");
+        }
         s_g = 0; gA++;
-        if (++s_c == KCH) { s_c = 0; sc_.next(s_ts); }
+        if (++s_c == KCH) { s_c = 0; sc_.step<PAIR>(s_ts, t_last); }
       }
     };
 
@@ -647,10 +690,12 @@
     TIM_FLUSH(20, 5);
   }
   tc_fence_before();
-  __syncthreads();
+  if (PAIR) cluster_sync_all();
+  else __syncthreads();
   if (warp == 1) {
     tc_fence_after();
-    asm volatile("tcgen05.dealloc.cta_group::1.sync.aligned.b32 %0, %1;" ::"r"(tmem_base), "r"(512u) : "memory");
+    if (PAIR) asm volatile("tcgen05.dealloc.cta_group::2.sync.aligned.b32 %0, %1;" ::"r"(tmem_base), "r"(512u) : "memory");
+    else asm volatile("tcgen05.dealloc.cta_group::1.sync.aligned.b32 %0, %1;" ::"r"(tmem_base), "r"(512u) : "memory");
   }
 }
 
@@ -666,6 +711,37 @@
   arb_conv_kernel<BN, MSUB, CONV2, T, POST, SB, PB><<<grid, kArbThreads, Cfg::SMEM, st>>>(*reinterpret_cast<const CUtensorMap*>(a.tmB), a);
 }
 
+template <bool CONV2>
+void launch_arb_pair_t(const ArbConvArgs& a, cudaStream_t st) {
+  using Cfg = ArbCfg<256, 1, false, true>;
+  auto kern = arb_conv_kernel<256, 1, CONV2, false, false, 0, false, true>;
+  cudaLaunchConfig_t cfg = {};
+  cfg.blockDim = dim3(kArbThreads, 1, 1); cfg.dynamicSmemBytes = Cfg::SMEM; cfg.stream = st;
+  cudaLaunchAttribute at[1];
+  at[0].id = cudaLaunchAttributeClusterDimension;
+  at[0].val.clusterDim.x = 2; at[0].val.clusterDim.y = 1; at[0].val.clusterDim.z = 1;
+  cfg.attrs = at; cfg.numAttrs = 1;
+  static DevOnce once;
+  static int max_clusters[64];
+  int dev = 0;
+  cudaGetDevice(&dev);
+  once.run(dev, [&] {
+    KKX_CUDA(cudaFuncSetAttribute(kern, cudaFuncAttributeMaxDynamicSharedMemorySize, (int)Cfg::SMEM));
+    int n = 0;
+    cfg.gridDim = dim3(2 * (device_sm_count(dev) / 2), 1, 1);
+    if (cudaOccupancyMaxActiveClusters(&n, kern, &cfg) != cudaSuccess || n <= 0) {
+      (void)cudaGetLastError();
+      n = device_sm_count(dev) / 2;
+    }
+    if (dev >= 0 && dev < 64) max_clusters[dev] = n;
+  });
+  int npairs = dev >= 0 && dev < 64 ? max_clusters[dev] : device_sm_count(dev) / 2;
+  const int units = (a.total_tiles + 1) / 2;
+  if (npairs > units) npairs = units;
+  cfg.gridDim = dim3((unsigned)(2 * npairs), 1, 1);
+  KKX_CUDA(cudaLaunchKernelEx(&cfg, kern, *reinterpret_cast<const CUtensorMap*>(a.tmB_pair), a));
+}
+
 }
 
 static int arb_variant(int C, int ks) {
@@ -678,6 +754,15 @@
 
 bool arb_conv_supported(int C, int ks, int dil, int B) {
   return (C == 128 || C == 256) && ks >= 1 && dil >= 1 && dil * (ks - 1) <= 50 && (ks & 1) && B <= kArbMaxB;
+}
+
+static bool arb_takes_pair(const ArbConvArgs& a) {
+  if (a.C != 256 || !a.tmB_pair || a.pair == 0) return false;
+  if (a.pair == 2) return true;
+  if (a.ks < (a.res ? 7 : 11)) return false;
+  int dev = 0;
+  cudaGetDevice(&dev);
+  return (a.total_tiles + 1) / 2 >= device_sm_count(dev) / 2;
 }
 
 void launch_arb_conv(const ArbConvArgs& a, cudaStream_t st) {
@@ -730,8 +815,13 @@
     else launch_arb_t<128, 2, false, true>(a, st);
   } else if (a.C == 128) {
     if (a.in_bf16) launch_arb_t<128, 2, true, false>(a, st); else launch_arb_t<128, 2, false, false>(a, st);
+  } else if (arb_takes_pair(a)) {
+    if (conv2) launch_arb_pair_t<true>(a, st); else launch_arb_pair_t<false>(a, st);
   } else {
-    if (a.in_bf16) launch_arb_t<256, 1, true, false>(a, st); else launch_arb_t<256, 1, false, false>(a, st);
+    static const bool pb256 = env_flag("KKX_ARB_PB256", true);
+    if (a.in_bf16) launch_arb_t<256, 1, true, false>(a, st);
+    else if (pb256) launch_arb_t<256, 1, false, false, false, 0, true>(a, st);
+    else launch_arb_t<256, 1, false, false>(a, st);
   }
   if (g_launch_stats && g_launch_stats->profile && g_launch_stats->detail) {
     char nm[96]; snprintf(nm, sizeof nm, "arb_conv[c%d k%d d%d %s%s m%lld]", a.C, a.ks, a.dil, conv2 ? "conv2" : "conv1", stream_bf ? " sb" : "", a.sum_m);
diff --git a/kokorox_b200/csrc/model.h b/kokorox_b200/csrc/model.h
--- a/kokorox_b200/csrc/model.h
+++ b/kokorox_b200/csrc/model.h
@@ -121,6 +121,7 @@
   int gemm_pair = 1;
   int fuse_planes = 1;
   int conv_pair = 1;
+  int arb_pair = 1;
   int fuse_noise_stats = 1;
   int ups_phase_loop = 3;
   int lstm_fast_gates = 1;
diff --git a/kokorox_b200/csrc/model_forward.cu b/kokorox_b200/csrc/model_forward.cu
--- a/kokorox_b200/csrc/model_forward.cu
+++ b/kokorox_b200/csrc/model_forward.cu
@@ -459,6 +459,7 @@
     base.tile_start = trows == 512 ? L.d_tiles512 : trows == 256 ? L.d_tiles256 : L.d_tiles128;
     base.total_tiles = trows == 512 ? L.ntiles512 : trows == 256 ? L.ntiles256 : L.ntiles128;
     base.scale = sc; base.shift = sh; base.nchunk = nch;
+    base.pair = opt.arb_pair ? 1 : 0;
     const bool sb = use_stream_bf16(C, k, B);
     void* xb0 = nullptr;
     if (sb && !x_bf16) xb0 = A.alloc_bytes((size_t)L.rows * C * 2);
@@ -473,6 +474,7 @@
       ArbConvArgs c1 = base;
       if (tim) c1.timing = tim + (C == 128 ? 0 : 64);
       c1.x = sb ? curb : (const void*)cur; c1.in_bf16 = sb ? 1 : 0; c1.alpha = w.a1[j]; c1.tmB = w.t1[j].tmap; c1.dil = dil[j];
+      c1.tmB_pair = w.t1[j].pair_map(C);
       c1.pad = dil[j] * (k - 1) / 2; c1.bias = w.b1[j];
       c1.out_bf16 = static_cast<__nv_bfloat16*>(abuf); c1.part = part;
       launch_arb_conv(c1, st);
@@ -481,6 +483,7 @@
       ArbConvArgs c2 = base;
       if (tim) c2.timing = tim + (C == 128 ? 32 : 96);
       c2.x = abuf; c2.in_bf16 = 1; c2.alpha = w.a2[j]; c2.tmB = w.t2[j].tmap; c2.dil = 1; c2.pad = (k - 1) / 2;
+      c2.tmB_pair = w.t2[j].pair_map(C);
       c2.bias = w.b2[j];
       if (sb) {
         c2.res = static_cast<const float*>(curb); c2.res_bf16 = 1;
diff --git a/kokorox_b200/csrc/testapi.cu b/kokorox_b200/csrc/testapi.cu
--- a/kokorox_b200/csrc/testapi.cu
+++ b/kokorox_b200/csrc/testapi.cu
@@ -472,8 +472,9 @@
 static int arb_conv_test(int device, const float* x, int B, const int* lens, int C, int in_bf16,
                          const float* scale, const float* shift, const float* alpha, const float* w,
                          const float* bias, int ks, int dil, const float* res, int res_bf16, float oscale,
-                         int accumulate, int want_bf16, float* out, float* sums, int desc_mode) {
-  return run(device, [&] {
+                         int accumulate, int want_bf16, float* out, float* sums, int desc_mode, int kernel = 0) {
+  return run(device, [&] {
+    if (kernel < 0 || kernel > 2) throw ArgError("kkx_test_arb_conv_pair: kernel must be 0, 1 or 2");
     if (!arb_conv_supported(C, ks, dil, B)) throw ArgError("kkx_test_arb_conv: unsupported shape");
     std::vector<int> off(B), tiles(B + 1, 0);
     const int MT = arb_tile_rows(C, ks);
@@ -511,6 +512,8 @@
     DevBuf doff(off.data(), B * 4), dlen(lens, B * 4), dts(tiles.data(), (B + 1) * 4);
     alignas(64) unsigned char tmB[128];
     make_tmap_bf16(tmB, dw.p, (long long)ks * C, C, (long long)ks * C, tc_box_n(C));
+    alignas(64) unsigned char tmBh[128];
+    if (C == 256) make_tmap_bf16(tmBh, dw.p, (long long)ks * C, C, (long long)ks * C, 128);
     ArbConvArgs a;
     a.x = dx.p; a.in_bf16 = in_bf16; a.scale = dsc.as<float>(); a.shift = dsh.as<float>(); a.alpha = dal.as<float>();
     a.tmB = tmB; a.C = C; a.ks = ks; a.dil = dil; a.pad = dil * (ks - 1) / 2;
@@ -520,6 +523,7 @@
     a.out_f32 = want_bf16 ? nullptr : dout.as<float>();
     a.res = res ? dres.as<float>() : nullptr; a.res_bf16 = res ? res_bf16 : 0; a.oscale = oscale; a.accumulate = accumulate;
     a.part = sums ? dpart.as<float>() : nullptr; a.nchunk = nchunk; (void)desc_mode;
+    a.tmB_pair = C == 256 ? tmBh : nullptr; a.pair = kernel == 1 ? 2 : kernel == 2 ? 1 : 0;
     launch_arb_conv(a, 0);
     KKX_CUDA(cudaDeviceSynchronize());
     if (want_bf16) {
@@ -558,6 +562,14 @@
                        want_bf16, out, sums, desc_mode);
 }
 
+KKX_API int kkx_test_arb_conv_pair(int device, const float* x, int B, const int* lens, int C, int in_bf16,
+                                   const float* scale, const float* shift, const float* alpha, const float* w,
+                                   const float* bias, int ks, int dil, const float* res, float oscale,
+                                   int accumulate, int want_bf16, float* out, float* sums, int kernel) {
+  return arb_conv_test(device, x, B, lens, C, in_bf16, scale, shift, alpha, w, bias, ks, dil, res, 0, oscale, accumulate,
+                       want_bf16, out, sums, 0, kernel);
+}
+
 KKX_API int kkx_test_arb_conv_stream(int device, const float* x, int B, const int* lens, int C, const float* scale,
                                      const float* shift, const float* alpha, const float* w, const float* bias, int ks,
                                      int dil, const float* res, float oscale, int accumulate, int want_bf16, float* out,
```

After: 10690, median of 6. About the same (-0.0%).
